# GiantAI/pixtrack

Hardware: AMD Instinct MI355X
Metric: tracked frames/sec at 640x480 (full NeRF render + UNet + LM loop) (higher is better)
Workload: dtype fp16 storage / fp32 accumulate (UNet, NeRF MLPs); fp32 (LM)

## Files before the change

include/pixtrack_hip.h:

```cpp
#ifndef PIXTRACK_HIP_H
#define PIXTRACK_HIP_H

#include <stdint.h>

#ifdef __cplusplus
extern "C" {
#endif

#define PXT_OK 0
#define PXT_E_ARG -1
#define PXT_E_HIP -2
#define PXT_E_TIMEOUT -3
#define PXT_E_STATE -4

#define PXT_MAX_LEVELS 8
#define PXT_LM_LOG_STRIDE 20

int pxt_version(void);
const char* pxt_last_error(void);
int pxt_device_cus(int* n_cus_host);

typedef struct {
  const float* fmap;
  const float* fref;
// ... 95 lines not shown
  float* out;
} pxt_lm_info_problem;
int64_t pxt_lm_information_workspace_bytes(int32_t n_problems);
int pxt_lm_information(const pxt_lm_info_problem* problems_host, int32_t n_problems, const pxt_lm_conf* conf_host,
                       void* workspace, void* stream);

#define PXT_LM_POINT_RECORD 8
#define PXT_LM_REPORT_SUMMARY 16
#define PXT_LM_REPORT_MAX_PROBLEMS 64
typedef struct {
  const float* p3d;
  const uint8_t* point_mask;
  int32_t n_points;
  pxt_lm_level level;
  const float* pose;
  int32_t pose_is_lm_record;
  float inlier_weight;
  float* points;
  float* summary;
} pxt_lm_report_problem;
int64_t pxt_lm_point_report_workspace_bytes(int32_t n_problems);
int pxt_lm_point_report(const pxt_lm_report_problem* problems_host, int32_t n_problems, const pxt_lm_conf* conf_host,
                        void* workspace, void* stream);

typedef struct pxt_unet pxt_unet;

int pxt_unet_create(const void* weights_host, int64_t n_bytes, pxt_unet** out_ctx);
int pxt_unet_destroy(pxt_unet* ctx);
int64_t pxt_unet_workspace_bytes(const pxt_unet* ctx, int32_t H, int32_t W);

int pxt_unet_activation_stats(pxt_unet* ctx, int32_t H, int32_t W, const void* workspace, float* stats_device ,
                              void* stream);

int pxt_unet_forward(pxt_unet* ctx, const void* image, int32_t image_is_u8, const uint8_t* mask,
                     int32_t H, int32_t W, float* const out_maps[3], const int32_t out_cstride[3],
                     int32_t normalize, void* workspace, void* stream);

#define PXT_UNET_MAX_BATCH 16
int64_t pxt_unet_workspace_bytes_batch(const pxt_unet* ctx, int32_t n_images, int32_t H, int32_t W);
int pxt_unet_forward_batch(pxt_unet* ctx, int32_t n_images, const void* const* images,
                           const int32_t* image_is_u8, const uint8_t* const* masks, int32_t H, int32_t W,
                           float* const* out_maps, const int32_t out_cstride[3], const int32_t* normalize,
                           void* workspace, void* stream);

int pxt_unet_set_tile_skip(pxt_unet* ctx, int32_t on);

int pxt_unet_set_batch_plan(pxt_unet* ctx, int32_t per_image_plan);

int64_t pxt_unet_workspace_bytes_pair(const pxt_unet* ctx, const int32_t H[2], const int32_t W[2]);
int pxt_unet_forward_pair(pxt_unet* ctx, const void* const* images, const int32_t* image_is_u8,
                          const uint8_t* const* masks, const int32_t H[2], const int32_t W[2],
                          float* const* out_maps, const int32_t out_cstride[3], const int32_t* normalize,
                          void* workspace, void* stream);
int pxt_unet_set_defer_join(pxt_unet* ctx, int32_t on);
int pxt_unet_pair_join(pxt_unet* ctx, void* stream);

int pxt_unet_create_f32(const void* weights_host, int64_t n_bytes, pxt_unet** out_ctx);
int pxt_unet_precision(const pxt_unet* ctx);


int pxt_conv3x3_nhwc_f16(const void* in, int32_t H, int32_t W, int32_t Cin, const void* weights,
                         const float* bias, int32_t Cout, int32_t relu, void* out, void* stream);

int pxt_conv3x3_nhwc_f32(const void* in, int32_t H, int32_t W, int32_t Cin, const void* weights,
                         const float* bias, int32_t Cout, int32_t relu, void* out, void* stream);

int64_t pxt_conv3x3_packed_bytes(int32_t Cin, int32_t Cout);
int pxt_conv3x3_pack_weights(const void* weights, int32_t Cin, int32_t Cout, void* packed, void* stream);
int pxt_conv3x3_packed(const void* in, int32_t H, int32_t W, int32_t Cin, const void* packed, const float* bias,
                       int32_t Cout, int32_t relu, void* out, void* pool_out, int32_t cfg, int32_t splits,
                       void* splitk_ws, int64_t splitk_ws_bytes, void* stream);

typedef struct pxt_ngp pxt_ngp;

typedef struct {
  int32_t n_levels, n_features, log2_hashmap, base_res;
  float per_level_scale;
  int32_t grid_cascades;
  float aabb_scale;
  float cone_angle;
  float depth_scale;
  int32_t linear_colors;
} pxt_ngp_model;

int pxt_ngp_create(const pxt_ngp_model* model_host, const void* grid_params_f16_host,
                   int64_t n_grid_params, const void* mlp_params_f16_host, int64_t n_mlp_params,
                   const uint8_t* occupancy_bits_host, int64_t n_occ_bytes, pxt_ngp** out_ctx);
int pxt_ngp_destroy(pxt_ngp* ctx);

typedef struct {
  float cam[12];
  float focal;
  float k1;
  float aabb_min[3], aabb_max[3];
  float background[4];
  float min_transmittance;
  int32_t width, height, spp;
  int32_t mode;
} pxt_ngp_view;

int pxt_ngp_render(pxt_ngp* ctx, const pxt_ngp_view* view_host, float* out_rgba,
                   uint64_t* stats ,
                   void* stream);

int pxt_ngp_render_both(pxt_ngp* ctx, const pxt_ngp_view* view_host, float* out_rgba, float* out_depth_rgba,
                        uint64_t* stats, void* stream);
// ... 77 lines not shown
```

pixtrack_amd/_lib.py:

```python
from __future__ import annotations

import ctypes as C
import os
from pathlib import Path
from typing import Optional

import torch

_HERE = Path(__file__).resolve().parent
LIB_PATH = Path(os.environ["PIXTRACK_HIP_LIB"]) if os.environ.get("PIXTRACK_HIP_LIB") else _HERE / "libpixtrack_hip.so"

PXT_MAX_LEVELS = 8
PXT_LM_LOG_STRIDE = 20
PXT_E_TIMEOUT = -3
ABI_VERSION = 13
PXT_LM_MAX_BATCH = 16
PXT_UNET_MAX_BATCH = 16
PXT_NGP_MAX_BATCH = 16
PXT_LM_INFO_RECORD = 48
PXT_LM_INFO_MAX_PROBLEMS = 64
PXT_LM_POINT_RECORD = 8
PXT_LM_REPORT_SUMMARY = 16
PXT_LM_REPORT_MAX_PROBLEMS = 64
PXT_POSE_ERR_RECORD = 8
# ... 8 lines not shown

class PxtError(RuntimeError):
    """Infrastructure failure of the native path (never a tracking failure)."""


class LmLevel(C.Structure):
    _fields_ = [
        ("fmap", C.c_void_p),
        ("fref", C.c_void_p),
        ("h", C.c_int32),
        ("w", C.c_int32),
        ("C", C.c_int32),
        ("cstride", C.c_int32),
        ("cam", C.c_float * 10),
        ("ndist", C.c_int32),
        ("lambda_", C.c_float * 6),
    ]


class LmConf(C.Structure):
    _fields_ = [
        ("num_iters", C.c_int32),
        ("pad", C.c_int32),
        ("loss", C.c_int32),
        ("loss_alpha", C.c_float),
        ("loss_scale", C.c_float),
        ("grad_stop", C.c_float),
        ("dt_stop", C.c_float),
        ("dR_stop", C.c_float),
        ("min_valid", C.c_int32),
        ("n_workgroups", C.c_int32),
        ("spin_limit", C.c_int32),
        ("path", C.c_int32),
    ]


class SampleLevel(C.Structure):
    _fields_ = [
        ("fmap", C.c_void_p),
        ("out", C.c_void_p),
        ("h", C.c_int32),
        ("w", C.c_int32),
        ("C", C.c_int32),
        ("cstride", C.c_int32),
        ("cam", C.c_float * 10),
        ("ndist", C.c_int32),
        ("x0", C.c_int32),
        ("y0", C.c_int32),
        ("full_w", C.c_int32),
        ("full_h", C.c_int32),
    ]


class NgpModel(C.Structure):
    _fields_ = [
        ("n_levels", C.c_int32),
        ("n_features", C.c_int32),
        ("log2_hashmap", C.c_int32),
        ("base_res", C.c_int32),
        ("per_level_scale", C.c_float),
        ("grid_cascades", C.c_int32),
        ("aabb_scale", C.c_float),
        ("cone_angle", C.c_float),
        ("depth_scale", C.c_float),
        ("linear_colors", C.c_int32),
    ]


class NgpView(C.Structure):
    _fields_ = [
        ("cam", C.c_float * 12),
        ("focal", C.c_float),
        ("k1", C.c_float),
        ("aabb_min", C.c_float * 3),
        ("aabb_max", C.c_float * 3),
        ("background", C.c_float * 4),
        ("min_transmittance", C.c_float),
        ("width", C.c_int32),
        ("height", C.c_int32),
        ("spp", C.c_int32),
        ("mode", C.c_int32),
    ]


class NgpOutputs(C.Structure):
    _fields_ = [("rgba", C.c_void_p), ("depth_rgba", C.c_void_p), ("rgb_u8", C.c_void_p), ("depth_nz", C.c_void_p)]


class LmCamera(C.Structure):
    _fields_ = [("conv27", C.c_double * 27), ("cam_slot", C.c_void_p * 2), ("cam_out13", C.c_void_p)]


class LmProblem(C.Structure):
    _fields_ = [("p3d", C.c_void_p), ("point_mask", C.c_void_p), ("n_points", C.c_int32),
                ("levels_host", C.POINTER(LmLevel)), ("n_levels", C.c_int32), ("T_init_host", C.POINTER(C.c_float)),
                ("out", C.c_void_p), ("log", C.c_void_p), ("workspace", C.c_void_p), ("cam_host", C.POINTER(LmCamera))]


class LmInfoProblem(C.Structure):
    _fields_ = [("p3d", C.c_void_p), ("point_mask", C.c_void_p), ("n_points", C.c_int32), ("level", LmLevel),
                ("pose", C.c_void_p), ("pose_is_lm_record", C.c_int32), ("out", C.c_void_p)]


class LmReportProblem(C.Structure):
    _fields_ = [("p3d", C.c_void_p), ("point_mask", C.c_void_p), ("n_points", C.c_int32), ("level", LmLevel),
                ("pose", C.c_void_p), ("pose_is_lm_record", C.c_int32), ("inlier_weight", C.c_float),
                ("points", C.c_void_p), ("summary", C.c_void_p)]


class RelocMap(C.Structure):
    _fields_ = [
        ("fmap", C.c_void_p),
        ("h", C.c_int32),
        ("w", C.c_int32),
        ("C", C.c_int32),
        ("cstride", C.c_int32),
        ("cam", C.c_float * 10),
        ("ndist", C.c_int32),
    ]


class RelocBank(C.Structure):
    _fields_ = [("p3d", C.c_void_p), ("fref", C.c_void_p), ("valid", C.c_void_p), ("n_points", C.c_int32)]


_lib: Optional[C.CDLL] = None

_VP, _I32, _I64 = C.c_void_p, C.c_int32, C.c_int64
PROTOTYPES = {
    "pxt_version": (C.c_int, []),
    "pxt_last_error": (C.c_char_p, []),
    "pxt_device_cus": (C.c_int, [C.POINTER(C.c_int)]),
    "pxt_lm_refine": (
        C.c_int,
        [_VP, _VP, _I32, C.POINTER(LmLevel), _I32, _VP, C.POINTER(LmConf), _VP, _VP, _VP, _VP],
    ),
    "pxt_lm_refine_cam": (
        C.c_int,
        [_VP, _VP, _I32, C.POINTER(LmLevel), _I32, _VP, C.POINTER(LmConf), _VP, _VP, _VP, C.POINTER(LmCamera), _VP],
    ),
    "pxt_lm_workspace_bytes": (_I64, []),
    "pxt_lm_batch_workspace_bytes": (_I64, [_I32]),
    "pxt_lm_refine_batch": (C.c_int, [C.POINTER(LmProblem), _I32, C.POINTER(LmConf), _VP, _VP]),
    "pxt_lm_information_workspace_bytes": (_I64, [_I32]),
    "pxt_lm_information": (C.c_int, [C.POINTER(LmInfoProblem), _I32, C.POINTER(LmConf), _VP, _VP]),
    "pxt_lm_point_report_workspace_bytes": (_I64, [_I32]),
    "pxt_lm_point_report": (C.c_int, [C.POINTER(LmReportProblem), _I32, C.POINTER(LmConf), _VP, _VP]),
    "pxt_sample_sparse": (C.c_int, [_VP, _I32, _VP, C.POINTER(SampleLevel), _I32, _I32, _I32, _VP, _VP]),
    "pxt_score_pose_hypotheses": (
        C.c_int, [C.POINTER(RelocMap), C.POINTER(RelocBank), _VP, _VP, _I32, C.POINTER(LmConf), _VP, _VP]),
    "pxt_unet_create": (C.c_int, [_VP, _I64, C.POINTER(_VP)]),
    "pxt_unet_create_f32": (C.c_int, [_VP, _I64, C.POINTER(_VP)]),
    "pxt_unet_precision": (C.c_int, [_VP]),
    "pxt_unet_destroy": (C.c_int, [_VP]),
    "pxt_unet_workspace_bytes": (_I64, [_VP, _I32, _I32]),
    "pxt_unet_forward": (
        C.c_int,
        [_VP, _VP, _I32, _VP, _I32, _I32, C.POINTER(_VP), C.POINTER(_I32), _I32, _VP, _VP],
    ),
    "pxt_unet_set_defer_join": (C.c_int, [_VP, _I32]),
    "pxt_unet_set_batch_plan": (C.c_int, [_VP, _I32]),
    "pxt_unet_set_tile_skip": (C.c_int, [_VP, _I32]),
    "pxt_unet_pair_join": (C.c_int, [_VP, _VP]),
    "pxt_unet_activation_stats": (C.c_int, [_VP, _I32, _I32, _VP, _VP, _VP]),
    "pxt_unet_workspace_bytes_batch": (_I64, [_VP, _I32, _I32, _I32]),
    "pxt_unet_forward_batch": (
        C.c_int,
        [_VP, _I32, C.POINTER(_VP), C.POINTER(_I32), C.POINTER(_VP), _I32, _I32, C.POINTER(_VP), C.POINTER(_I32),
         C.POINTER(_I32), _VP, _VP],
    ),
    "pxt_unet_workspace_bytes_pair": (_I64, [_VP, C.POINTER(_I32), C.POINTER(_I32)]),
    "pxt_unet_forward_pair": (
        C.c_int,
        [_VP, C.POINTER(_VP), C.POINTER(_I32), C.POINTER(_VP), C.POINTER(_I32), C.POINTER(_I32), C.POINTER(_VP),
         C.POINTER(_I32), C.POINTER(_I32), _VP, _VP],
    ),
    "pxt_conv3x3_nhwc_f16": (C.c_int, [_VP, _I32, _I32, _I32, _VP, _VP, _I32, _I32, _VP, _VP]),
    "pxt_conv3x3_nhwc_f32": (C.c_int, [_VP, _I32, _I32, _I32, _VP, _VP, _I32, _I32, _VP, _VP]),
    "pxt_conv3x3_packed_bytes": (_I64, [_I32, _I32]),
    "pxt_conv3x3_pack_weights": (C.c_int, [_VP, _I32, _I32, _VP, _VP]),
    "pxt_conv3x3_packed": (C.c_int, [_VP, _I32, _I32, _I32, _VP, _VP, _I32, _I32, _VP, _VP, _I32, _I32, _VP, _I64, _VP]),
    "pxt_ngp_create": (C.c_int, [C.POINTER(NgpModel), _VP, _I64, _VP, _I64, _VP, _I64, C.POINTER(_VP)]),
    "pxt_ngp_destroy": (C.c_int, [_VP]),
    "pxt_ngp_render": (C.c_int, [_VP, C.POINTER(NgpView), _VP, _VP, _VP]),
    "pxt_ngp_render_both": (C.c_int, [_VP, C.POINTER(NgpView), _VP, _VP, _VP, _VP]),
    "pxt_ngp_render_both_from_pose": (C.c_int, [_VP, C.POINTER(NgpView), _VP, C.POINTER(C.c_double), _VP, _VP, _VP, _VP, _VP]),
    "pxt_ngp_render_frame": (C.c_int, [_VP, C.POINTER(NgpView), _I32, _I32, C.POINTER(NgpOutputs), _VP, _VP]),
    "pxt_ngp_camera_slot": (_VP, [_VP]),
    "pxt_ngp_batch_workspace_bytes": (_I64, [_I32]),
    "pxt_ngp_render_frame_batch": (C.c_int, [C.POINTER(_VP), C.POINTER(NgpView), _I32, C.POINTER(_I32), _I32,
                                              C.POINTER(NgpOutputs), C.POINTER(_VP), _VP, _VP]),
    "pxt_ngp_create_shared": (C.c_int, [_VP, C.POINTER(_VP)]),
    "pxt_ngp_timing_enable": (C.c_int, [_VP, _I32]),
    "pxt_ngp_timing_read": (C.c_int, [_VP, C.POINTER(C.c_float), C.POINTER(_I32)]),
    "pxt_ngp_query": (C.c_int, [_VP, _VP, _VP, _I32, _VP, _VP]),
    "pxt_depth_mask": (C.c_int, [_VP, _I32, _I32, _I32, _I32, _VP, _VP, _VP]),
    "pxt_depth_mask_plane": (C.c_int, [_VP, _I32, _I32, _I32, _I32, _VP, _VP, _VP]),
    "pxt_rgba_to_u8": (C.c_int, [_VP, _I32, _I32, C.c_float, _VP, _VP]),
    "pxt_resize_linear": (C.c_int, [_VP, _I32, _I32, _I32, _VP, _I32, _I32, _VP]),
    "pxt_resize_activity": (C.c_int, [_VP, _VP, _I32, _I32, _I32, _I32, _VP, _VP]),
    "pxt_points_from_depth_workspace_bytes": (_I64, [_I32, _I32]),
    "pxt_points_from_depth": (C.c_int, [_VP, _I32, _I32, C.POINTER(C.c_float), C.c_float, C.c_float, C.c_float, _I32, _I32,
                                        _VP, _VP, _VP, _VP, _VP]),
    "pxt_pose_errors_workspace_bytes": (_I64, [_I32, _I32]),
    "pxt_pose_errors": (C.c_int, [_VP, _I32, _VP, _I32, _I32, _VP, _VP, _VP]),
    "pxt_depth_agreement_workspace_bytes": (_I64, [_I32, _I32, _I32]),
    "pxt_depth_agreement": (C.c_int, [_VP, _VP, _I32, _I32, _I32, C.c_float, C.POINTER(C.c_float), _I32, _VP, _VP, _VP]),
    "pxt_symmetric_pose_errors_workspace_bytes": (_I64, [_I32, _I32, _I32]),
    "pxt_symmetric_pose_errors": (C.c_int, [_VP, _I32, _VP, _I32, _VP, _I32, _VP, _VP, _VP]),
    "pxt_sensor_vsd_workspace_bytes": (_I64, [_I32, _I32, _I32]),
    "pxt_sensor_vsd": (C.c_int, [_VP, _VP, _VP, _VP, _I32, _I32, _I32, _I32, _I32, C.c_float, C.c_float, C.c_float,
                                 C.POINTER(C.c_float), _I32, _VP, _VP, _VP]),
# ... 56 lines not shown
```

pixtrack_amd/csrc/pxt_common.h:

```cpp
#pragma once

#include <hip/hip_runtime.h>
#include <stdint.h>

#include "../../include/pixtrack_hip.h"

#define PXT_WAVE 64

namespace pxt {

void set_last_error(const char* what, hipError_t e);
hipStream_t shared_side_stream(int i);
#define PXT_HIP_CHECK(expr)                         \
  do {                                              \
    hipError_t _e = (expr);                         \
    if (_e != hipSuccess) {                         \
      ::pxt::set_last_error(#expr, _e);             \
      return PXT_E_HIP;                             \
    }                                               \
  } while (0)

struct Cam {
  float w, h, fx, fy, cx, cy, k1, k2, p1, p2;
  int ndist;
};

__host__ __device__ inline Cam make_cam(const float* c10, int ndist) {
  Cam c;
  c.w = c10[0]; c.h = c10[1]; c.fx = c10[2]; c.fy = c10[3]; c.cx = c10[4]; c.cy = c10[5];
  c.k1 = c10[6]; c.k2 = c10[7]; c.p1 = c10[8]; c.p2 = c10[9];
  c.ndist = ndist;
  return c;
}

constexpr float kCamEps = 1e-3f;

__device__ inline bool project_point(const Cam& c, float x, float y, float z, float& u, float& v,
                                     float* J ) {
  bool visible = z > kCamEps;
  float zc = fmaxf(z, kCamEps);
  float iz = 1.0f / zc;
  float xn = x * iz, yn = y * iz;
  float xd = xn, yd = yn;
  bool dist_ok = true;
  float Jd00 = 1.f, Jd01 = 0.f, Jd10 = 0.f, Jd11 = 1.f;
  if (c.ndist > 0) {
    float r2 = xn * xn + yn * yn;
    float radial = c.k1 * r2 + c.k2 * r2 * r2;
    xd = xn + xn * radial;
    yd = yn + yn * radial;
    float disc = 9.f * c.k1 * c.k1 - 20.f * c.k2;
    bool limited = ((c.k2 > 0.f) && (disc > 0.f)) || ((c.k2 <= 0.f) && (c.k1 > 0.f));
    if (limited) {
      float limit = (c.k2 > 0.f) ? (sqrtf(fmaxf(disc, 0.f)) - 3.f * c.k1) / (10.f * c.k2)
                                 : 1.f / (3.f * c.k1);
      dist_ok = r2 < fabsf(limit);
    }
    float uv = xn * yn;
    float d_radial = 2.f * c.k1 + 4.f * c.k2 * r2;
    Jd00 += radial + xn * xn * d_radial;
    Jd11 += radial + yn * yn * d_radial;
    Jd01 += uv * d_radial;
    Jd10 += uv * d_radial;
    if (c.ndist > 2) {
      xd += 2.f * c.p1 * uv + c.p2 * (r2 + 2.f * xn * xn);
      yd += 2.f * c.p2 * uv + c.p1 * (r2 + 2.f * yn * yn);
      Jd00 += 2.f * c.p1 * yn + 6.f * c.p2 * xn;
      Jd11 += 2.f * c.p2 * xn + 6.f * c.p1 * yn;
      Jd01 += 2.f * c.p1 * xn + 2.f * c.p2 * yn;
      Jd10 += 2.f * c.p2 * yn + 2.f * c.p1 * xn;
    }
  }
  u = xd * c.fx + c.cx;
  v = yd * c.fy + c.cy;
  bool in_img = (u >= 0.f) && (v >= 0.f) && (u <= c.w - 1.f) && (v <= c.h - 1.f);
  if (J) {
    float a = iz, bx = -x * iz * iz, by = -y * iz * iz;
    float m00 = c.fx * Jd00, m01 = c.fx * Jd01, m10 = c.fy * Jd10, m11 = c.fy * Jd11;
    J[0] = m00 * a; J[1] = m01 * a; J[2] = m00 * bx + m01 * by;
    J[3] = m10 * a; J[4] = m11 * a; J[5] = m10 * bx + m11 * by;
  }
  return visible && dist_ok && in_img;
}

template <int WIDTH>
__device__ inline float group_allreduce_sum(float v) {
#pragma unroll
  for (int m = 1; m < WIDTH; m <<= 1) v += __shfl_xor(v, m, PXT_WAVE);
  return v;
}
// ... 113 lines not shown
```

pixtrack_amd/csrc/pxt_conv_v2.h:

```cpp
#pragma once

#include <type_traits>

namespace pxt {

constexpr int kV2RowBytes = 1280;
constexpr int kV2Cols = 18;

struct FusedHead {
  const half8* wfrag;
  const float* conf_w;
  const float* bias;
  float* out[PXT_UNET_MAX_BATCH];
  int normalize[PXT_UNET_MAX_BATCH];
  int cstride, enabled;
};

struct FusedFirst {
  const void* image[PXT_UNET_MAX_BATCH];
  const uint8_t* mask[PXT_UNET_MAX_BATCH];
  int is_u8[PXT_UNET_MAX_BATCH];
  const float* w;
  const float* b;
  int enabled;
};

struct TileSkip {
  const uint8_t* flags;
  const half_t* value;
};

template <int TH, int BNC, int NT>
__device__ __forceinline__ void conv_fill_constant_tile(const half_t* __restrict__ value, half_t* __restrict__ out_img,
                                                        half_t* __restrict__ pool_img, int H, int W, int Cout, int ty0, int tx0,
                                                        int co0) {
  constexpr int CH = BNC / 8;
  const half8* cv = (const half8*)(value + co0);
  for (int i = threadIdx.x; i < TH * 16 * CH; i += NT) {
    const int c = i % CH, p = i / CH;
    const int y = ty0 + (p >> 4), x = tx0 + (p & 15);
    if (y < H && x < W) *(half8*)(out_img + ((size_t)y * W + x) * Cout + co0 + 8 * c) = cv[c];
  }
  if (pool_img) {
    const int Hp = H >> 1, Wp = W >> 1;
    for (int i = threadIdx.x; i < (TH / 2) * 8 * CH; i += NT) {
      const int c = i % CH, p = i / CH;
      const int y = (ty0 >> 1) + (p >> 3), x = (tx0 >> 1) + (p & 7);
      if (y < Hp && x < Wp) *(half8*)(pool_img + ((size_t)y * Wp + x) * Cout + co0 + 8 * c) = cv[c];
    }
  }
}

struct ConvArgs {
  const half_t* in;
  int H, W, Cin;
  const half_t* wpk;
  const float* bias;
  int Cout, relu;
  half_t* out;
  float* partial;
  UpSrc up;
  half_t* pool;
  FusedHead head;
  FusedFirst first;
  TileSkip skip;
};

__host__ __device__ inline size_t packed_weight_index(int cout, int tap, int cin, int Cout) {
  const int k = cin & 31, s = k >> 4, lane = (cout & 31) + 32 * ((k & 15) >> 3), j = k & 7;
  return ((((size_t)(cin >> 5) * 9 + tap) * 2 + s) * (size_t)(Cout >> 5) + (cout >> 5)) * 512 + lane * 8 + j;
}

__global__ void pack_conv_weights_kernel(const half_t* __restrict__ w , int Cin, int Cout,
                                         half_t* __restrict__ packed) {
  const long long i = (long long)blockIdx.x * blockDim.x + threadIdx.x;
  if (i >= (long long)Cout * 9 * Cin) return;
  const int cin = (int)(i % Cin);
  const int tap = (int)((i / Cin) % 9);
  const int cout = (int)(i / ((long long)Cin * 9));
  packed[packed_weight_index(cout, tap, cin, Cout)] = w[i];
}

typedef __attribute__((ext_vector_type(2))) _Float16 half2v;

template <int I, int N, class F>
__device__ __forceinline__ void static_for(F&& f) {
  if constexpr (I < N) {
    f(std::integral_constant<int, I>{});
    static_for<I + 1, N>(f);
  }
}

__device__ inline int opaque(int x) {
  asm volatile("" : "+v"(x));
  return x;
}

__device__ inline unsigned pool2x2_pk(unsigned v) {
  auto sw = __builtin_amdgcn_permlane16_swap(v, v, false, false);
  half2v a = __builtin_bit_cast(half2v, (unsigned)sw[0]), b = __builtin_bit_cast(half2v, (unsigned)sw[1]);
  half2v m = __builtin_elementwise_max(a, b);
  const unsigned mu = __builtin_bit_cast(unsigned, m);
  const unsigned nb = (unsigned)__builtin_amdgcn_update_dpp((int)mu, (int)mu, 0xB1 , 0xF, 0xF, false);
  m = __builtin_elementwise_max(m, __builtin_bit_cast(half2v, nb));
  return __builtin_bit_cast(unsigned, m);
}

#if PXT_EXP_STAMPS
__device__ unsigned long long pxt_stamps[8192 * 16];
#define PXT_STAMP(k)                                                                              \
  do {                                                                                            \
    if (threadIdx.x == 0) {                                                                       \
      const unsigned wg_ = blockIdx.x + gridDim.x * (blockIdx.y + gridDim.y * blockIdx.z);        \
      if (wg_ < 8192) pxt_stamps[wg_ * 16 + (k)] = __builtin_amdgcn_s_memtime();                 \
      if (wg_ < 8192 && ((k) == 0 || (k) == 3))                                                   \
        pxt_stamps[wg_ * 16 + ((k) == 0 ? 14 : 15)] = __builtin_amdgcn_s_memrealtime();          \
    }                                                                                             \
  } while (0)
#else
#define PXT_STAMP(k)
#endif
template <int CW, int PBW, int WC, int WP, bool UPCAT, int AR = 3, bool FIRST = false>
__global__ __launch_bounds__(256, AR > 3 ? 1 : 2) void conv3x3_v2_kernel(const ConvArgs a) {
  static_assert(!FIRST || !UPCAT, "the fused first layer feeds a plain layer");
  static_assert(18 % AR == 0, "the ring is indexed by the step modulo AR at compile time");
  static_assert(WC * WP == 4, "four waves per workgroup");
  constexpr int TH = 2 * PBW * WP, HR = TH + 2;
  constexpr int BNC = 32 * CW * WC;
  constexpr int kElems = HR * kV2Cols * 4;
  constexpr int KH = (kElems + 255) / 256;
  constexpr int NB = 2;
  constexpr int KB = (KH + NB - 1) / NB;
  constexpr int kBuf = HR * kV2RowBytes;
  extern __shared__ __attribute__((aligned(16))) char smem[];

  PXT_STAMP(0);
  const int tid = threadIdx.x;
  const int lane = tid & 63;
  const int wave = __builtin_amdgcn_readfirstlane(tid >> 6);
  const int wc = wave / WP, wp = wave % WP;
  const int H = a.H, W = a.W, Cin = a.Cin, Cout = a.Cout;
  const int tiles_x = (W + 15) >> 4;
  const int tiles_per = tiles_x * ((H + TH - 1) / TH);
  const int img = blockIdx.x / tiles_per, tile = blockIdx.x % tiles_per;
  const int n_img = gridDim.x / tiles_per;
  const int ty0 = (tile / tiles_x) * TH, tx0 = (tile % tiles_x) * 16;
  const int co0 = blockIdx.y * BNC;
  const int Cs = UPCAT ? Cin - a.up.Cp : Cin;
  const int in_w = UPCAT ? a.up.Ws : W;
  const half_t* in = a.in + (size_t)img * (UPCAT ? a.up.Hs : H) * in_w * Cs;
  const half_t* prev = UPCAT ? a.up.prev + (size_t)img * a.up.Hp * a.up.Wp * a.up.Cp : nullptr;
  if (a.skip.flags != nullptr && a.skip.flags[blockIdx.x] == 0) {
    conv_fill_constant_tile<TH, BNC, 256>(a.skip.value, a.out + (size_t)img * H * W * Cout,
                                          a.pool ? a.pool + (size_t)img * (H >> 1) * (W >> 1) * Cout : nullptr, H, W, Cout, ty0,
                                          tx0, co0);
    return;
  }

  float* const s_bias = (float*)(smem + 2 * kBuf + (UPCAT ? (PBW * WP + 2) * 10 * 64 : 0));
  if (tid < BNC) s_bias[tid] = a.bias[co0 + tid];

  f32x16 acc[CW][PBW];
#pragma unroll
  for (int c = 0; c < CW; ++c)
#pragma unroll
    for (int p = 0; p < PBW; ++p)
#pragma unroll
      for (int r = 0; r < 16; ++r) acc[c][p][r] = 0.f;

  const int r31 = lane & 31, khalf = lane >> 5;
  int boff[3][2];
#pragma unroll
  for (int kx = 0; kx < 3; ++kx)
#pragma unroll
    for (int s = 0; s < 2; ++s) {
      const int col = (r31 & 15) + kx;
      boff[kx][s] = (2 * PBW * wp + (r31 >> 4)) * kV2RowBytes + col * 64 + (((2 * s + khalf) ^ ((col >> 2) & 3)) << 4);
    }

  const int n_chunks = Cin >> 5;
  const int per_z = (n_chunks + (int)gridDim.z - 1) / (int)gridDim.z;
  const int ch_begin = (int)blockIdx.z * per_z, ch_end = min(n_chunks, ch_begin + per_z);

  const size_t a_step = (size_t)(Cout >> 5) * 512;
  const half_t* aptr = a.wpk + ((size_t)ch_begin * 18) * a_step + (size_t)((co0 >> 5) + CW * wc) * 512 + lane * 8;

  half8 r_in[KB];
  unsigned goff[KH];
#pragma unroll
  for (int k = 0; k < KH; ++k) {
    const int i = tid + 256 * k;
    const int pix = i >> 2, seg = i & 3;
    const int gy = ty0 + pix / kV2Cols - 1, gx = tx0 + pix % kV2Cols - 1;
    const bool ok = i < kElems && gy >= 0 && gy < H && gx >= 0 && gx < W;
    goff[k] = ok ? ((unsigned)(gy * in_w + gx) * (unsigned)Cs + (unsigned)(seg * 8)) * 2u : 0x80000000u;
  }
  const __amdgpu_buffer_rsrc_t in_rsrc = __builtin_amdgcn_make_buffer_rsrc(
      (void*)in, 0, (int)((size_t)(UPCAT ? a.up.Hs : H) * in_w * Cs * 2), 0x00020000);
  const int cp0 = UPCAT ? a.up.Cp : 0;
  auto halo_issue = [&](int c0, int batch) {
#pragma unroll
    for (int kk = 0; kk < KB; ++kk) {
      const int k = batch * KB + kk;
      if (k < KH)
        r_in[kk] = __builtin_bit_cast(half8, __builtin_amdgcn_raw_buffer_load_b128(
                                                 in_rsrc, (int)(goff[k] + (unsigned)((c0 - cp0) * 2)), 0, 0));
    }
  };
  auto halo_write = [&](int buf, int batch) {
    const int t_ = opaque(tid);
#pragma unroll
    for (int kk = 0; kk < KB; ++kk) {
      const int k = batch * KB + kk;
      const int i = t_ + 256 * k;
      const int pix = i >> 2, seg = i & 3;
      const int hy = pix / kV2Cols, hx = pix % kV2Cols;
      if (k < KH && i < kElems)
        *(half8*)(smem + buf * kBuf + hy * kV2RowBytes + hx * 64 + ((seg ^ ((hx >> 2) & 3)) << 4)) = r_in[kk];
    }
  };

  constexpr int PH = TH / 2 + 2, PW = 10;
  constexpr int kPatchElems = PH * PW * 4, KP = (kPatchElems + 255) / 256;
  static_assert(!UPCAT || KP <= KB, "the patch pieces reuse the halo staging registers");
  char* const patch = smem + 2 * kBuf;
  unsigned poff[UPCAT ? KP : 1], up_src[UPCAT ? KH : 1];
  if (UPCAT) {
    const int py0 = (ty0 >> 1) - 1, px0 = (tx0 >> 1) - 1;
#pragma unroll
    for (int kp = 0; kp < KP; ++kp) {
      const int i = min(tid + 256 * kp, kPatchElems - 1);
      const int pp = i >> 2, seg = i & 3;
      const int sy = min(max(py0 + pp / PW, 0), a.up.Hp - 1), sx = min(max(px0 + pp % PW, 0), a.up.Wp - 1);
      poff[kp] = (unsigned)(sy * a.up.Wp + sx) * (unsigned)a.up.Cp + (unsigned)(seg * 8);
    }
#pragma unroll
    for (int k = 0; k < KH; ++k) {
      const int i = tid + 256 * k;
      const int pix = i >> 2, seg = i & 3;
      const int gy = ty0 + pix / kV2Cols - 1, gx = tx0 + pix % kV2Cols - 1;
      const bool ok = i < kElems && gy >= 0 && gy < H && gx >= 0 && gx < W;
      const float sy = fmaxf(((float)gy + 0.5f) * 0.5f - 0.5f, 0.f);
      const float sx = fmaxf(((float)gx + 0.5f) * 0.5f - 0.5f, 0.f);
      const int y0 = min((int)sy, a.up.Hp - 1), x0 = min((int)sx, a.up.Wp - 1);
      const int y1 = min(y0 + 1, a.up.Hp - 1), x1 = min(x0 + 1, a.up.Wp - 1);
      const float ay = sy - (float)y0, ax = sx - (float)x0;
      const int pidx = ok ? (y0 - py0) * PW + (x0 - px0) : 0;
      up_src[k] = ((unsigned)(pidx * 64 + seg * 16) << 8) | (ok ? 64u : 0u) | (x1 != x0 ? 1u : 0u) | (y1 != y0 ? 2u : 0u) |
                  (ax == 0.25f ? 4u : ax == 0.75f ? 8u : 0u) | (ay == 0.25f ? 16u : ay == 0.75f ? 32u : 0u);
    }
  }
  auto patch_issue = [&](int c0) {
#pragma unroll
    for (int kp = 0; kp < KP; ++kp) r_in[kp] = *(const half8*)(prev + (poff[UPCAT ? kp : 0] + (unsigned)c0));
  };
  auto patch_write = [&]() {
    const int t_ = opaque(tid);
#pragma unroll
    for (int kp = 0; kp < KP; ++kp) {
      const int i = t_ + 256 * kp;
      if (i < kPatchElems) *(half8*)(patch + i * 16) = r_in[kp];
    }
  };
  auto patch_interp = [&](int buf) {
    const int t_ = opaque(tid);
#pragma unroll
    for (int k = 0; k < KH; ++k) {
      const int i = t_ + 256 * k;
      const int pix = i >> 2, seg = i & 3;
      const int hy = pix / kV2Cols, hx = pix % kV2Cols;
      const unsigned f = (unsigned)opaque((int)up_src[UPCAT ? k : 0]);
      const char* src = patch + (f >> 8);
      const int dx = (f & 1u) ? 64 : 0, dy = (f & 2u) ? PW * 64 : 0;
      const float ax = (f & 4u) ? 0.25f : (f & 8u) ? 0.75f : 0.f;
      const float ay = (f & 16u) ? 0.25f : (f & 32u) ? 0.75f : 0.f;
      const half8 p00 = *(const half8*)(src), p01 = *(const half8*)(src + dx);
      const half8 p10 = *(const half8*)(src + dy), p11 = *(const half8*)(src + dy + dx);
      const bool ok_ = (f & 64u) != 0;
      const half_t wa = (half_t)(ok_ ? (1.f - ax) * (1.f - ay) : 0.f), wb = (half_t)(ok_ ? ax * (1.f - ay) : 0.f);
      const half_t wc = (half_t)(ok_ ? (1.f - ax) * ay : 0.f), wd = (half_t)(ok_ ? ax * ay : 0.f);
      half8 v = p00 * wa;
// ... 287 lines not shown
```

pixtrack_amd/csrc/pxt_conv_v3.h:

```cpp
#pragma once

namespace pxt {

template <int KC>
struct V3Geo {
  static constexpr int kPix = KC * 2;
  static constexpr int kNP = KC / 8;
  static constexpr int kRow = 20 * kPix;
  static constexpr int kPixPerBankRow = 256 / kPix;
  __device__ static inline int swz(int col) {
    return kPixPerBankRow == 4 ? ((col >> 2) & 3) : ((col >> 3) & 1);
  }
};

__host__ __device__ inline size_t packed_weight_index_v3(int cout, int tap, int cin, int Cout) {
  const int ky = tap / 3, kx = tap % 3;
  const int k = cin & 31, s = k >> 4, lane = (cout & 31) + 32 * ((k & 15) >> 3), j = k & 7;
  const size_t group = (size_t)(cin >> 5) * 6 + s * 3 + kx;
  return ((group * 3 + ky) * (size_t)(Cout >> 5) + (cout >> 5)) * 512 + lane * 8 + j;
}

__global__ void pack_conv_weights_v3_kernel(const half_t* __restrict__ w , int Cin, int Cout,
                                            half_t* __restrict__ packed) {
  const long long i = (long long)blockIdx.x * blockDim.x + threadIdx.x;
// ... 4 lines not shown
  packed[packed_weight_index_v3(cout, tap, cin, Cout)] = w[i];
}

__device__ inline unsigned pk_max(unsigned a, unsigned b) {
  return __builtin_bit_cast(unsigned, __builtin_elementwise_max(__builtin_bit_cast(half2v, a), __builtin_bit_cast(half2v, b)));
}

constexpr int v3_lds_bytes(int CW, int PBW, int WC, int WP, int KC, bool upcat = false, int KS = 1) {
  return KS * (2 * (2 * PBW * WP + 2) * (20 * KC * 2) + 2 * 3 * CW * WC * 1024) + 32 * CW * WC * 4 +
         (upcat ? (PBW * WP + 2) * 10 * KC * 2 : 0);
}

template <int CW, int PBW, int WC, int WP, int KC, bool UPCAT = false, int KS = 1>
__global__ __launch_bounds__(256 * KS, 2) void conv3x3_v3_kernel(const ConvArgs a) {
  static_assert(WC * WP == 4, "four waves per quartet");
  static_assert(KS == 1 || (KS == 2 && !UPCAT), "K split across two wave quartets: plain layers only");
  static_assert(KC == 16 || KC == 32, "chunk of 16 or 32 input channels");
  using G = V3Geo<KC>;
  constexpr int TH = 2 * PBW * WP, HR = TH + 2;
  constexpr int NCB = CW * WC, BNC = 32 * NCB;
  constexpr int NG = 3 * (KC / 16);
  constexpr int kBuf = HR * G::kRow;
  constexpr int kABuf = 3 * NCB * 1024;
  constexpr int kElems = HR * kV2Cols * G::kNP;
  constexpr int KH = (kElems + 255) / 256;
  constexpr int kAElems = 3 * NCB * 64;
  constexpr int KA = (kAElems + 255) / 256;
  extern __shared__ __attribute__((aligned(16))) char smem[];
  constexpr int kQuartet = 2 * kBuf + 2 * kABuf;
  const int kh = KS == 1 ? 0 : __builtin_amdgcn_readfirstlane((int)threadIdx.x >> 8);
  char* const s_halo = smem + kh * kQuartet;
  char* const s_a = s_halo + 2 * kBuf;
  float* const s_bias = (float*)(smem + KS * kQuartet);
  char* const patch = smem + KS * kQuartet + BNC * 4;

  PXT_STAMP(0);
  const int tid = threadIdx.x & 255;
  const int lane = tid & 63;
  const int wave = __builtin_amdgcn_readfirstlane(tid >> 6);
  const int wc = wave / WP, wp = wave % WP;
  const int H = a.H, W = a.W, Cin = a.Cin, Cout = a.Cout;
  const int tiles_x = (W + 15) >> 4;
  const int tiles_per = tiles_x * ((H + TH - 1) / TH);
  const int img = blockIdx.x / tiles_per, tile = blockIdx.x % tiles_per;
  const int n_img = gridDim.x / tiles_per;
  const int ty0 = (tile / tiles_x) * TH, tx0 = (tile % tiles_x) * 16;
  const int co0 = blockIdx.y * BNC;
  const int Cs = UPCAT ? Cin - a.up.Cp : Cin;
  const int in_w = UPCAT ? a.up.Ws : W;
  const int cp0 = UPCAT ? a.up.Cp : 0;
  const half_t* in = a.in + (size_t)img * (UPCAT ? a.up.Hs : H) * in_w * Cs;
  const half_t* prev = UPCAT ? a.up.prev + (size_t)img * a.up.Hp * a.up.Wp * a.up.Cp : nullptr;
  if (a.skip.flags != nullptr && a.skip.flags[blockIdx.x] == 0) {
    conv_fill_constant_tile<TH, BNC, 256 * KS>(a.skip.value, a.out + (size_t)img * H * W * Cout,
                                               a.pool ? a.pool + (size_t)img * (H >> 1) * (W >> 1) * Cout : nullptr, H, W, Cout,
                                               ty0, tx0, co0);
    return;
  }

  if ((int)threadIdx.x < BNC) s_bias[threadIdx.x] = a.bias[co0 + threadIdx.x];

  f32x16 acc[CW][PBW];
#pragma unroll
  for (int c = 0; c < CW; ++c)
#pragma unroll
    for (int p = 0; p < PBW; ++p)
#pragma unroll
      for (int r = 0; r < 16; ++r) acc[c][p][r] = 0.f;

  const int r31 = lane & 31, khalf = lane >> 5;
  const int lrow = 2 * PBW * wp + (r31 >> 4) * PBW, lcol = r31 & 15;

  const int n_chunks = Cin / KC;
  const int per_z = (n_chunks + (int)gridDim.z - 1) / (int)gridDim.z;
  int ch_begin = (int)blockIdx.z * per_z, ch_end = min(n_chunks, ch_begin + per_z);
  if (KS == 2) {
    const int half = (ch_end - ch_begin) >> 1;
    ch_begin += kh * half;
    ch_end = ch_begin + half;
  }
  const int n_groups = (ch_end - ch_begin) * NG;

  const size_t a_group = (size_t)3 * (Cout >> 5) * 512;
  const half_t* const wbase = a.wpk + (size_t)ch_begin * NG * a_group + (size_t)(co0 >> 5) * 512;
  unsigned a_src[KA];
#pragma unroll
  for (int k = 0; k < KA; ++k) {
    const int i = min(tid + 256 * k, kAElems - 1);
    const int ky = i / (NCB * 64), rem = i % (NCB * 64);
    a_src[k] = (unsigned)(ky * (Cout >> 5) * 512 + rem * 8);
  }
  half8 r_a[KA];
  const half_t* a_next = wbase;
  auto a_issue_piece = [&](auto k_c) {
    constexpr int k = decltype(k_c)::value;
    r_a[k] = *(const half8*)(a_next + a_src[k]);
  };
  auto a_write_piece = [&](auto k_c, int buf) {
    constexpr int k = decltype(k_c)::value;
    const int i = opaque(tid) + 256 * k;
    if (i < kAElems) *(half8*)(s_a + buf * kABuf + i * 16) = r_a[k];
  };

  half8 r_in[KH];
  unsigned goff[KH];
#pragma unroll
  for (int k = 0; k < KH; ++k) {
    const int i = tid + 256 * k;
    const int pix = i / G::kNP, seg = i % G::kNP;
    const int gy = ty0 + pix / kV2Cols - 1, gx = tx0 + pix % kV2Cols - 1;
    const bool ok = i < kElems && gy >= 0 && gy < H && gx >= 0 && gx < W;
    goff[k] = ok ? ((unsigned)(gy * in_w + gx) * (unsigned)Cs + (unsigned)(seg * 8)) * 2u : 0x80000000u;
  }
  const __amdgpu_buffer_rsrc_t in_rsrc = __builtin_amdgcn_make_buffer_rsrc(
      (void*)in, 0, (int)((size_t)(UPCAT ? a.up.Hs : H) * in_w * Cs * 2), 0x00020000);
  auto halo_issue_piece = [&](auto k_c, int c0) {
    constexpr int k = decltype(k_c)::value;
    r_in[k] = __builtin_bit_cast(half8, __builtin_amdgcn_raw_buffer_load_b128(in_rsrc, (int)(goff[k] + (unsigned)((c0 - cp0) * 2)), 0, 0));
  };
  auto halo_write_piece = [&](auto k_c, int buf) {
    constexpr int k = decltype(k_c)::value;
    const int i = opaque(tid) + 256 * k;
    const int pix = i / G::kNP, seg = i % G::kNP;
    const int hy = pix / kV2Cols, hx = pix % kV2Cols;
    if (i < kElems) *(half8*)(s_halo + buf * kBuf + hy * G::kRow + hx * G::kPix + ((seg ^ G::swz(hx)) << 4)) = r_in[k];
  };

  constexpr int PH = TH / 2 + 2, PW = 10;
  constexpr int kPatchElems = PH * PW * G::kNP, KP = (kPatchElems + 255) / 256;
  static_assert(!UPCAT || KP <= KH, "the patch pieces reuse the halo staging registers");
  unsigned poff[UPCAT ? KP : 1], up_src[UPCAT ? KH : 1];
  if constexpr (UPCAT) {
    const int py0 = (ty0 >> 1) - 1, px0 = (tx0 >> 1) - 1;
#pragma unroll
    for (int kp = 0; kp < KP; ++kp) {
      const int i = min(tid + 256 * kp, kPatchElems - 1);
      const int pp = i / G::kNP, seg = i % G::kNP;
      const int sy = min(max(py0 + pp / PW, 0), a.up.Hp - 1), sx = min(max(px0 + pp % PW, 0), a.up.Wp - 1);
      poff[kp] = (unsigned)(sy * a.up.Wp + sx) * (unsigned)a.up.Cp + (unsigned)(seg * 8);
    }
#pragma unroll
    for (int k = 0; k < KH; ++k) {
      const int i = tid + 256 * k;
      const int pix = i / G::kNP, seg = i % G::kNP;
      const int gy = ty0 + pix / kV2Cols - 1, gx = tx0 + pix % kV2Cols - 1;
      const bool ok = i < kElems && gy >= 0 && gy < H && gx >= 0 && gx < W;
      const float sy = fmaxf(((float)gy + 0.5f) * 0.5f - 0.5f, 0.f);
      const float sx = fmaxf(((float)gx + 0.5f) * 0.5f - 0.5f, 0.f);
      const int y0 = min((int)sy, a.up.Hp - 1), x0 = min((int)sx, a.up.Wp - 1);
      const int y1 = min(y0 + 1, a.up.Hp - 1), x1 = min(x0 + 1, a.up.Wp - 1);
      const float ay = sy - (float)y0, ax = sx - (float)x0;
      const int pidx = ok ? (y0 - py0) * PW + (x0 - px0) : 0;
      up_src[k] = ((unsigned)(pidx * G::kPix + seg * 16) << 8) | (ok ? 64u : 0u) | (x1 != x0 ? 1u : 0u) | (y1 != y0 ? 2u : 0u) |
                  (ax == 0.25f ? 4u : ax == 0.75f ? 8u : 0u) | (ay == 0.25f ? 16u : ay == 0.75f ? 32u : 0u);
    }
  }
  auto patch_issue_piece = [&](auto k_c, int c0) {
    constexpr int k = decltype(k_c)::value;
    if constexpr (UPCAT && k < KP) r_in[k] = *(const half8*)(prev + (poff[k] + (unsigned)c0));
  };
  auto patch_write_piece = [&](auto k_c) {
    constexpr int k = decltype(k_c)::value;
    if constexpr (UPCAT && k < KP) {
      const int i = opaque(tid) + 256 * k;
      if (i < kPatchElems) *(half8*)(patch + i * 16) = r_in[k];
    }
  };
  auto patch_interp_piece = [&](auto k_c, int buf) {
    constexpr int k = decltype(k_c)::value;
    if constexpr (UPCAT) {
      const int i = opaque(tid) + 256 * k;
      const int pix = i / G::kNP, seg = i % G::kNP;
      const int hy = pix / kV2Cols, hx = pix % kV2Cols;
      const unsigned f = (unsigned)opaque((int)up_src[k]);
      const char* src = patch + (f >> 8);
      const int dx = (f & 1u) ? G::kPix : 0, dy = (f & 2u) ? PW * G::kPix : 0;
      const float ax = (f & 4u) ? 0.25f : (f & 8u) ? 0.75f : 0.f;
      const float ay = (f & 16u) ? 0.25f : (f & 32u) ? 0.75f : 0.f;
      const half8 p00 = *(const half8*)(src), p01 = *(const half8*)(src + dx);
      const half8 p10 = *(const half8*)(src + dy), p11 = *(const half8*)(src + dy + dx);
      const bool ok_ = (f & 64u) != 0;
      const half_t wa = (half_t)(ok_ ? (1.f - ax) * (1.f - ay) : 0.f), wb = (half_t)(ok_ ? ax * (1.f - ay) : 0.f);
      const half_t wc = (half_t)(ok_ ? (1.f - ax) * ay : 0.f), wd = (half_t)(ok_ ? ax * ay : 0.f);
      half8 v = p00 * wa;
      v = p01 * wb + v;
      v = p10 * wc + v;
// ... 282 lines not shown
```

pixtrack_amd/csrc/pxt_lm.hip:

```cpp
#include "pxt_common.h"
#include "pxt_lm_point.h"

#include <algorithm>

namespace pxt {

constexpr int kLmBlock = 512;
constexpr int kLmWaves = kLmBlock / PXT_WAVE;
constexpr int kLmMaxGrid = 256;
constexpr int kNAcc = 32;
constexpr int kGrpStride = 33;
constexpr unsigned kSpinLimit = 1u << 22;

struct LmLevelDev {
  const float* fmap;
  const float* fref;
  int h, w, C, cs;
  float cam[10];
  int ndist;
  float lambda[6];
};

struct LmGrid {
  int G, b;
// ... 656 lines not shown
        __hip_atomic_store(&P.cam_out[12], 1.f, __ATOMIC_RELEASE, __HIP_MEMORY_SCOPE_SYSTEM);
      }
    }
  }
}

__global__ __launch_bounds__(kLmBlock) void lm_refine_kernel(const LmParams P) {
  __shared__ LmShared sh;
  lm_refine_problem(P, LmGrid{(int)gridDim.x, (int)blockIdx.x}, sh);
}

__global__ __launch_bounds__(kLmBlock) void lm_refine_batch_kernel(const LmParams* __restrict__ params, const int K,
                                                                   const int contiguous) {
  __shared__ LmShared sh;
  const int G = (int)gridDim.x / K;
  const int p = contiguous ? (int)blockIdx.x / G : (int)blockIdx.x % K;
  const int b = contiguous ? (int)blockIdx.x % G : (int)blockIdx.x / K;
  lm_refine_problem(params[p], LmGrid{G, b}, sh);
}

struct SampleLevelDev {
  const float* fmap;
  float* out;
  int h, w, C, cs;
  float cam[10];
  int ndist;
  int x0, y0, fw, fh;
};

struct SampleParams {
  const float* p3d;
  float T[12];
  int n, n_levels, pad, normalize;
  SampleLevelDev lv[PXT_MAX_LEVELS];
  uint8_t* valid;
};

template <int LG>
__device__ inline bool sample_level(const SampleParams& P, const SampleLevelDev& L, int n,
                                    bool active, float px, float py, float pz, int sub) {
  const Cam cam = make_cam(L.cam, L.ndist);
  const int W = L.w, H = L.h, C = L.C, cs = L.cs;
  const int FW = L.fw, FH = L.fh;
  const float pad = (float)P.pad;
  float u = 0.f, v = 0.f;
  bool valid = active;
  point_in_window(cam, px, py, pz, valid, FW, FH, pad, u, v, nullptr);
  if (!active) return false;
  float* o = L.out + (size_t)n * cs;
  if (!valid) {
    for (int c0 = 4 * sub; c0 < cs; c0 += 4 * LG) *(float4*)(o + c0) = make_float4(0, 0, 0, 0);
    return false;
  }
  const float fu = floorf(u), fv = floorf(v);
  const int ix0f = (int)fu, iy0f = (int)fv;
  const float ax = u - fu, ay = v - fv;
  const int x1f = min(ix0f + 1, FW - 1), y1f = min(iy0f + 1, FH - 1);
  const float mx = (ix0f + 1 < FW) ? 1.f : 0.f, my = (iy0f + 1 < FH) ? 1.f : 0.f;
  const float w00 = (1.f - ax) * (1.f - ay), w10 = ax * (1.f - ay) * mx, w01 = (1.f - ax) * ay * my,
              w11 = ax * ay * mx * my;
  const int ix0 = min(max(ix0f - L.x0, 0), W - 1), iy0 = min(max(iy0f - L.y0, 0), H - 1);
  const int x1 = min(max(x1f - L.x0, 0), W - 1), y1 = min(max(y1f - L.y0, 0), H - 1);
  const float* p00 = L.fmap + ((size_t)iy0 * W + ix0) * cs;
  const float* p10 = L.fmap + ((size_t)iy0 * W + x1) * cs;
  const float* p01 = L.fmap + ((size_t)y1 * W + ix0) * cs;
  const float* p11 = L.fmap + ((size_t)y1 * W + x1) * cs;
  float ss = 0.f;
  for (int c0 = 4 * sub; c0 < C; c0 += 4 * LG) {
    float4 a = *(const float4*)(p00 + c0), b = *(const float4*)(p10 + c0),
           c = *(const float4*)(p01 + c0), d = *(const float4*)(p11 + c0);
    float4 f;
    f.x = w00 * a.x + w10 * b.x + w01 * c.x + w11 * d.x;
    f.y = w00 * a.y + w10 * b.y + w01 * c.y + w11 * d.y;
    f.z = w00 * a.z + w10 * b.z + w01 * c.z + w11 * d.z;
    f.w = w00 * a.w + w10 * b.w + w01 * c.w + w11 * d.w;
    ss += f.x * f.x + f.y * f.y + f.z * f.z + f.w * f.w;
    *(float4*)(o + c0) = f;
  }
  ss = group_allreduce_sum<LG>(ss);
  if (P.normalize) {
    const float inv = 1.f / fmaxf(sqrtf(ss), 1e-12f);
    for (int c0 = 4 * sub; c0 < C; c0 += 4 * LG) {
      float4 f = *(float4*)(o + c0);
      f.x *= inv; f.y *= inv; f.z *= inv; f.w *= inv;
      *(float4*)(o + c0) = f;
    }
  }
  if (sub == 0) {
    o[C] = w00 * p00[C] + w10 * p10[C] + w01 * p01[C] + w11 * p11[C];
    for (int c = C + 1; c < cs; ++c) o[c] = 0.f;
  }
  return true;
}

__global__ __launch_bounds__(256) void sample_sparse_kernel(const SampleParams P) {
  constexpr int LG = 32;
  constexpr int GPW = PXT_WAVE / LG;
  const int lane = threadIdx.x & (PXT_WAVE - 1);
  const int sub = lane % LG, grp = lane / LG;
  const int wave_global = (blockIdx.x * blockDim.x + threadIdx.x) / PXT_WAVE;
  const int n = wave_global * GPW + grp;
  const bool active = n < P.n;
  float X = 0.f, Y = 0.f, Z = 1.f;
  if (active) {
    X = P.p3d[3 * n];
    Y = P.p3d[3 * n + 1];
    Z = P.p3d[3 * n + 2];
  }
  float px, py, pz;
  transform_point(P.T, X, Y, Z, px, py, pz);
  bool all_valid = active;
  for (int l = 0; l < P.n_levels; ++l)
    all_valid = sample_level<LG>(P, P.lv[l], n, active, px, py, pz, sub) && all_valid;
  if (active && sub == 0) P.valid[n] = all_valid ? 1 : 0;
}
// ... 185 lines not shown
```

pixtrack_amd/csrc/pxt_lm_point.h:

```cpp
#pragma once

#include "pxt_common.h"

namespace pxt {

__device__ inline void robust_loss(int kind, float alpha, float scale, float x, float& loss,
                                   float& w) {
  if (kind == 0) {
    loss = x;
    w = 1.f;
    return;
  }
  float a2 = scale * scale;
  float y = x / a2;
  float l, d;
  if (kind == 1) {
    if (y <= 1.f) {
      l = y;
      d = 1.f;
    } else {
      float sy = sqrtf(y);
      l = 2.f * sy - 1.f;
      d = fmaxf(1.1920929e-07f, 1.f / sy);
    }
// ... 3 lines not shown
      d = 2.f / (y + 2.f);
    } else if (alpha == 2.f) {
      l = y;
      d = 1.f;
    } else {
      float beta = fmaxf(fabsf(alpha - 2.f), 1e-7f);
      float as = (alpha >= 0.f ? 1.f : -1.f) * fmaxf(fabsf(alpha), 1e-7f);
      l = 2.f * (beta / as) * (powf(y / beta + 1.f, 0.5f * alpha) - 1.f);
      d = powf(y / beta + 1.f, 0.5f * alpha - 1.f);
    }
  }
  loss = l * a2;
  w = d;
}

__device__ inline float lm_dpp_add(float v, int ctrl_tag) {
  const int iv = __builtin_bit_cast(int, v);
  int o;
  if (ctrl_tag == 0) o = __builtin_amdgcn_update_dpp(iv, iv, 0xB1, 0xF, 0xF, false);
  else if (ctrl_tag == 1) o = __builtin_amdgcn_update_dpp(iv, iv, 0x4E, 0xF, 0xF, false);
  else if (ctrl_tag == 2) o = __builtin_amdgcn_update_dpp(iv, iv, 0x141, 0xF, 0xF, false);
  else o = __builtin_amdgcn_update_dpp(iv, iv, 0x140, 0xF, 0xF, false);
  return v + __builtin_bit_cast(float, o);
}

__device__ inline float lm_group_sum(float v, bool wide) {
  v = lm_dpp_add(v, 0);
  v = lm_dpp_add(v, 1);
  v = lm_dpp_add(v, 2);
  if (wide) {
    v = lm_dpp_add(v, 3);
    v += __shfl_xor(v, 16, PXT_WAVE);
  }
  return v;
}

template <int LG>
__device__ inline float lm_group_sum_t(float v) {
  v = lm_dpp_add(v, 0);
  v = lm_dpp_add(v, 1);
  v = lm_dpp_add(v, 2);
  if (LG >= 16) v = lm_dpp_add(v, 3);
  if (LG >= 32) v += __shfl_xor(v, 16, PXT_WAVE);
  return v;
}

__device__ inline float lm_row16_sum(float v) {
  v = lm_dpp_add(v, 0);
  v = lm_dpp_add(v, 1);
  v = lm_dpp_add(v, 2);
  return lm_dpp_add(v, 3);
}

__device__ inline void transform_point(const float* T, float X, float Y, float Z, float& px, float& py, float& pz) {
  px = T[0] * X + T[1] * Y + T[2] * Z + T[9];
  py = T[3] * X + T[4] * Y + T[5] * Z + T[10];
  pz = T[6] * X + T[7] * Y + T[8] * Z + T[11];
}

__device__ inline void point_in_window(const Cam& cam, float px, float py, float pz, bool& valid, int W, int H, float pad,
                                       float& u, float& v, float* Jw ) {
  valid = project_point(cam, px, py, pz, u, v, Jw) && valid;
  valid = valid && (u >= pad) && (v >= pad) && (u <= (float)(W - 1) - pad) && (v <= (float)(H - 1) - pad);
}

__device__ inline void bilinear_weights(float u, float v, int& ix0, int& iy0, float& w00, float& w10, float& w01,
                                        float& w11) {
  const float fu = floorf(u), fv = floorf(v);
  ix0 = (int)fu;
  iy0 = (int)fv;
  const float ax = u - fu, ay = v - fv;
  w00 = (1.f - ax) * (1.f - ay);
  w10 = ax * (1.f - ay);
  w01 = (1.f - ax) * ay;
  w11 = ax * ay;
}

#define PXT_LM_POINT_CH(w00_, w10_, w01_, w11_, a01_, a02_, a10_, a11_, a12_, a13_, a20_, a21_, a22_, a23_, a31_, a32_, \
                        f_, s_cost_, A0_, A1_, B00_, B01_, B11_)                                                        \
  {                                                                                                                     \
    const float a01 = (a01_), a02 = (a02_), a10 = (a10_), a11 = (a11_), a12 = (a12_), a13 = (a13_), a20 = (a20_),       \
                a21 = (a21_), a22 = (a22_), a23 = (a23_), a31 = (a31_), a32 = (a32_);                                   \
    const float F = (w00_) * a11 + (w10_) * a12 + (w01_) * a21 + (w11_) * a22;                                          \
    const float Fxp = (w00_) * a12 + (w10_) * a13 + (w01_) * a22 + (w11_) * a23;                                        \
    const float Fxm = (w00_) * a10 + (w10_) * a11 + (w01_) * a20 + (w11_) * a21;                                        \
    const float Fyp = (w00_) * a21 + (w10_) * a22 + (w01_) * a31 + (w11_) * a32;                                        \
    const float Fym = (w00_) * a01 + (w10_) * a02 + (w01_) * a11 + (w11_) * a12;                                        \
    const float gx = 0.5f * (Fxp - Fxm), gy = 0.5f * (Fyp - Fym);                                                       \
    const float r = F - (f_);                                                                                           \
    (s_cost_) += r * r;                                                                                                 \
    (A0_) += r * gx;                                                                                                    \
    (A1_) += r * gy;                                                                                                    \
    (B00_) += gx * gx;                                                                                                  \
    (B01_) += gx * gy;                                                                                                  \
    (B11_) += gy * gy;                                                                                                  \
  }

#define PXT_LM_POINT_CH_COST(w00_, w10_, w01_, w11_, a11_, a12_, a21_, a22_, f_, s_cost_)    \
  {                                                                                          \
    const float a11 = (a11_), a12 = (a12_), a21 = (a21_), a22 = (a22_);                      \
    const float F = (w00_) * a11 + (w10_) * a12 + (w01_) * a21 + (w11_) * a22;               \
    const float r = F - (f_);                                                                \
    (s_cost_) += r * r;                                                                      \
  }

__device__ inline void point_jacobian(const float* Jw, float px, float py, float pz, float* J0, float* J1) {
  J0[0] = Jw[0]; J0[1] = Jw[1]; J0[2] = Jw[2];
  J1[0] = Jw[3]; J1[1] = Jw[4]; J1[2] = Jw[5];
  J0[3] = -Jw[1] * pz + Jw[2] * py;
  J0[4] = Jw[0] * pz - Jw[2] * px;
  J0[5] = -Jw[0] * py + Jw[1] * px;
  J1[3] = -Jw[4] * pz + Jw[5] * py;
  J1[4] = Jw[3] * pz - Jw[5] * px;
  J1[5] = -Jw[3] * py + Jw[4] * px;
}

template <bool ADD>
__device__ __forceinline__ void point_normal_terms(float* dst, float wgt, const float* J0, const float* J1, float A0,
                                                   float A1, float B00, float B01, float B11) {
  float M0[6], M1[6];
#pragma unroll
  for (int k = 0; k < 6; ++k) {
    M0[k] = B00 * J0[k] + B01 * J1[k];
    M1[k] = B01 * J0[k] + B11 * J1[k];
    dst[k] = (ADD ? dst[k] : 0.f) + wgt * (J0[k] * A0 + J1[k] * A1);
  }
  int idx = 6;
#pragma unroll
// ... 7 lines not shown
```

pixtrack_amd/csrc/pxt_unet.hip:

```cpp
#include "pxt_common.h"
#include "pxt_unet_f32.h"

#include <algorithm>
#include <array>
#include <cstdio>
#include <cstdlib>
#include <cstring>
#include <utility>
#include <vector>

namespace pxt {

typedef _Float16 half_t;
typedef __attribute__((ext_vector_type(8))) _Float16 half8;
typedef __attribute__((ext_vector_type(4))) _Float16 half4;
typedef __attribute__((ext_vector_type(16))) float f32x16;

constexpr int kNumConv = 17;
constexpr int kNumHeads = 3;

constexpr int kFW = 64, kFH = 4;
struct FirstImages {
  const void* image[PXT_UNET_MAX_BATCH];
  const uint8_t* mask[PXT_UNET_MAX_BATCH];
  int is_u8[PXT_UNET_MAX_BATCH];
};

template <int COUT>
__global__ __launch_bounds__(256) void conv_first_kernel(const FirstImages imgs, int H, int W,
                                                         const float* __restrict__ wts,
                                                         const float* __restrict__ bias,
                                                         half_t* __restrict__ out) {
  __shared__ float s_px[(kFH + 2) * (kFW + 2) * 3];
  __shared__ __attribute__((aligned(16))) half_t s_out[kFH * kFW * COUT];
  const int im = blockIdx.y;
  const void* image = imgs.image[im];
  const uint8_t* mask = imgs.mask[im];
  const bool u8 = imgs.is_u8[im] != 0;
  out += (size_t)im * H * W * COUT;
  const int tiles_x = (W + kFW - 1) / kFW;
  const int tx0 = (blockIdx.x % tiles_x) * kFW, ty0 = (blockIdx.x / tiles_x) * kFH;
  const float mean[3] = {0.485f, 0.456f, 0.406f};
  const float istd[3] = {1.f / 0.229f, 1.f / 0.224f, 1.f / 0.225f};
  for (int i = threadIdx.x; i < (kFH + 2) * (kFW + 2); i += 256) {
    const int hy = i / (kFW + 2), hx = i % (kFW + 2);
    const int yy = ty0 + hy - 1, xx = tx0 + hx - 1;
    const bool ok = yy >= 0 && yy < H && xx >= 0 && xx < W;
    float m = 1.f;
    if (ok && mask) m = (float)mask[(size_t)yy * W + xx];
#pragma unroll
    for (int c = 0; c < 3; ++c) {
      float v = 0.f;
      if (ok) {
// ... 282 lines not shown
      else for (int x = 0; x < n; ++x) any |= p[x];
    } else {
      const uint8_t* p = u8 + ((size_t)y * W + x0) * 3;
      if (n == 8 && (((uintptr_t)p) & 7) == 0) {
        const unsigned long long* q = (const unsigned long long*)p;
        any = (q[0] | q[1] | q[2]) != 0ull;
      } else {
        for (int x = 0; x < 3 * n; ++x) any |= p[x];
      }
    }
  }
  any |= __shfl_xor(any, 1, 64);
  any |= __shfl_xor(any, 2, 64);
  any |= __shfl_xor(any, 4, 64);
  if (live && r == 0) grid[(size_t)img * bh * bw + b] = any ? 1 : 0;
}

struct SkipLayerGeo {
  int th, shift, radius, h, w, offset;
};
struct SkipGeo {
  SkipLayerGeo l[6];
  int n_layers;
};
__global__ void skip_tile_flags_kernel(const SkipGeo geo, const uint8_t* __restrict__ grid, int H, int W, int bh, int bw,
                                       int n_img, uint8_t* __restrict__ flags) {
  const SkipLayerGeo g = geo.l[blockIdx.y];
  const int tiles_x = (g.w + 15) >> 4, tiles_y = (g.h + g.th - 1) / g.th;
  const int t = (blockIdx.x * blockDim.x + threadIdx.x) >> 6, lane = threadIdx.x & 63;
  if (t >= n_img * tiles_x * tiles_y) return;
  const int img = t / (tiles_x * tiles_y), tile = t % (tiles_x * tiles_y);
  const int ty0 = (tile / tiles_x) * g.th, tx0 = (tile % tiles_x) * 16;
  const int y0 = (ty0 << g.shift) - g.radius, y1 = (min(ty0 + g.th, g.h) << g.shift) + g.radius;
  const int x0 = (tx0 << g.shift) - g.radius, x1 = (min(tx0 + 16, g.w) << g.shift) + g.radius;
  unsigned any = (y0 < 0 || x0 < 0 || y1 > H || x1 > W) ? 1u : 0u;
  if (!any) {
    const uint8_t* gi = grid + (size_t)img * bh * bw;
    const int by0 = y0 >> 3, bx0 = x0 >> 3, nby = ((y1 - 1) >> 3) - by0 + 1, nbx = ((x1 - 1) >> 3) - bx0 + 1;
    for (int c = lane; c < nby * nbx; c += 64) any |= gi[(by0 + c / nbx) * bw + bx0 + c % nbx];
  }
  any = __ballot(any != 0) != 0ull;
  if (lane == 0) flags[g.offset + t] = any ? 1 : 0;
}

__global__ void skip_fill_kernel(half_t* __restrict__ dst, int n_pix, int C, const half_t* __restrict__ value) {
  const int i = blockIdx.x * blockDim.x + threadIdx.x;
  if (i < n_pix * C) dst[i] = value[i % C];
}
__global__ void skip_copy_kernel(half_t* __restrict__ dst, const half_t* __restrict__ src, int C) {
  const int i = blockIdx.x * blockDim.x + threadIdx.x;
  if (i < C) dst[i] = src[i];
}

struct UnetLayer {
  int cin, cout;
  const void* w;
  const float* b;
};

}

struct pxt_unet {
  pxt::UnetF32* f32 = nullptr;
  void* dev_head = nullptr;
  const pxt::half_t* head_w[pxt::kNumHeads];
  const float* head_b[pxt::kNumHeads];
  void* dev_blob = nullptr;
  void* dev_head0 = nullptr;
  void* dev_packed = nullptr;
  const pxt::half_t* conv_packed[pxt::kNumConv];
  int64_t n_bytes = 0;
  struct SideSet {
    hipStream_t side = nullptr;
    hipEvent_t ev_enc4 = nullptr, ev_dec1 = nullptr, ev_side = nullptr;
  } sides[2];
  hipStream_t pass2 = nullptr;
  hipEvent_t ev_fork = nullptr, ev_join = nullptr;
  struct SkipEntry {
    int cfg[6] = {0, 0, 0, 0, 0, 0};
    unsigned long long stamp = 0;
    pxt::half_t* values = nullptr;
  } skip_cache[8];
  unsigned long long skip_clock = 0;
  bool tile_skip = true;
  void* skip_scratch = nullptr;
  bool plan_as_single = false;
  bool defer_join = false;
  bool join_pending = false;
  pxt::UnetLayer conv[pxt::kNumConv];
  pxt::UnetLayer head[pxt::kNumHeads];
};

using namespace pxt;

namespace {

inline int env_int(const char* name, int dflt) { const char* e = getenv(name); return e ? atoi(e) : dflt; }
std::vector<std::array<int, 3>> parse_plan(const char* e) {
  std::vector<std::array<int, 3>> v;
  for (; e && *e; e = strchr(e, ';') ? strchr(e, ';') + 1 : nullptr) {
    std::array<int, 3> t = {0, 0, 0};
    if (sscanf(e, "%d:%d:%d", &t[0], &t[1], &t[2]) >= 2) v.push_back(t);
  }
  return v;
}
struct Knobs {
  int streams = env_int("PXT_UNET_STREAMS", 2);
  bool merge_heads = env_int("PXT_UNET_MERGE_HEADS", 1) != 0;
  bool skip = env_int("PXT_UNET_SKIP", 1) != 0;
  bool fuse_first = env_int("PXT_UNET_FUSE_FIRST", 1) != 0;
  const char* plan_env = getenv("PXT_CONV_PLAN");
  std::vector<std::array<int, 3>> plan = parse_plan(plan_env);
  bool debug = getenv("PXT_CONV_DEBUG") != nullptr;
};
const Knobs& knobs() { static const Knobs k; return k; }

struct EncBlock { int first, n, cin, c; };
constexpr int kNumEncLayers = 13;
constexpr EncBlock kEnc[5] = {{0, 2, 3, 64}, {2, 2, 64, 128}, {4, 3, 128, 256}, {7, 3, 256, 512}, {10, 3, 512, 512}};
inline int enc_block(int li) { int b = 4; while (kEnc[b].first > li) --b; return b; }
inline bool enc_last(int li) { return li == kEnc[enc_block(li)].first + kEnc[enc_block(li)].n - 1; }

inline bool fuses_first(const pxt_unet* ctx) { return knobs().fuse_first && ctx->conv[1].cin == 64 && ctx->conv[1].cout == 64; }

struct TileCfg {
  int kernel;
  int CW, PBW, WC, WP, KC, KS;
  int upcat_c;
  bool pool;
  int twin;
  bool deep;
  bool first;
};
constexpr int kNumCfgs = 22;
constexpr TileCfg kTileCfgs[kNumCfgs] = {
    {},
    {2, 2, 4, 2, 2, 32, 1, 0, true, 0, true, false},
    {2, 2, 2, 1, 4, 32, 1, 64, true, 0, false, true},
    {},
    {2, 2, 2, 2, 2, 32, 1, 0, true, 0, false, false},
    {},
    {2, 1, 2, 1, 4, 32, 1, 32, true, 0, false, false},
    {}, {}, {}, {},
    {3, 2, 4, 2, 2, 32, 1, 0, true, 0, false, false},
    {},
    {3, 2, 4, 1, 4, 16, 1, 0, true, 0, false, false},
    {3, 2, 2, 2, 2, 32, 1, 0, true, 0, false, false},
    {3, 2, 3, 2, 2, 32, 1, 0, false, 0, false, false},
    {3, 1, 4, 1, 4, 16, 1, 32, true, 0, false, false},
    {3, 2, 3, 1, 4, 16, 1, 64, false, 0, false, false},
    {3, 2, 3, 2, 2, 32, 2, 0, false, 15, false, false},
    {3, 2, 4, 2, 2, 32, 2, 0, true, 11, false, false},
    {3, 1, 2, 1, 4, 16, 1, 32, true, 0, false, false},
    {3, 2, 2, 1, 4, 16, 1, 64, true, 0, false, false}};
inline bool cfg_valid(int cfg) { return cfg >= 1 && cfg < kNumCfgs && kTileCfgs[cfg].kernel != 0; }
inline int cfg_th(int cfg) { return 2 * kTileCfgs[cfg].PBW * kTileCfgs[cfg].WP; }
inline int cfg_bnc(int cfg) { return 32 * kTileCfgs[cfg].CW * kTileCfgs[cfg].WC; }
inline const half_t* cfg_taps(int cfg, const half_t* wpk, int cin, int cout) {
  return kTileCfgs[cfg].kernel == 3 ? wpk + (size_t)cout * 9 * cin : wpk;
}

struct ConvPlan { int cfg, tiles, nb, splits; };

// ... 14 lines not shown
                   int force_splits, bool upcat, bool wants_pool) {
  ConvPlan P;
  const int plan_img = sc.single ? 1 : n_img, plan_peers = sc.single ? 2 : sc.peers;
  auto wgs_of = [&](int cfg) {
    const int th = cfg_th(cfg);
    return plan_peers * plan_img * ((H + th - 1) / th) * ((W + 15) / 16) * (cout / cfg_bnc(cfg));
  };
  int cfg = force_cfg;
  if (!cfg_valid(cfg) || cout % cfg_bnc(cfg) != 0) {
    if (cout % 128 == 0) {
      cfg = wgs_of(4) >= 512 ? 4 : 1;
      const int w15 = wgs_of(15);
      if (!wants_pool && w15 >= 192 && w15 <= 512) cfg = 15;
      const bool even_k = (cin / 32) % 2 == 0;
      if (cfg == 15 && w15 <= 256 && even_k) cfg = 18;
      if (cfg == 1 && wgs_of(1) <= 256 && wgs_of(1) >= 128 && even_k) cfg = 19;
      if (cfg == 1 && allow_split && wgs_of(15) < 192 && (cin / 32) % 8 == 0) cfg = 18;
    }
    else if (cout % 64 == 0) cfg = 2;
    else cfg = 6;
  }
  if (cfg_valid(cfg) && kTileCfgs[cfg].KS == 2 && (upcat || (cin / 32) % 2 != 0)) cfg = kTileCfgs[cfg].twin;
  P.cfg = cfg;
  const int th = cfg_th(cfg);
  P.tiles = n_img * ((H + th - 1) / th) * ((W + 15) / 16);
  P.nb = cout / cfg_bnc(cfg);
  const int plan_tiles = P.tiles / n_img * plan_img;
  P.splits = allow_split ? (force_splits > 0 ? std::min(force_splits, std::max(1, cin / 32)) : choose_splits(plan_peers * plan_tiles * P.nb, cin / 32, upcat, plan_tiles * P.nb)) : 1;
  if (kTileCfgs[cfg].KS == 2) {
    while (P.splits > 1 && (cin / 32) % (2 * P.splits) != 0) --P.splits;
  }
  return P;
}

inline int upcat_cfg(int cout, int H, int W) {
  return cout % 64 == 0 ? ((long long)H * W >= 120 * 160 ? 21 : 2) : 20;
}

size_t splitk_bytes(int n_img, int H, int W, int cin, int cout, bool upcat = false) {
  int splits = 1;
  for (int single = 0; single < 2; ++single)
    for (int peers = 1; peers <= 2; ++peers)
      for (int pool = 0; pool < (upcat ? 1 : 2); ++pool)
        splits = std::max(splits, plan_conv(PlanScope{peers, single != 0, 0}, n_img, H, W, cin, cout, true,
                                            upcat ? upcat_cfg(cout, H, W) : 0, 0, upcat, pool != 0).splits);
  return splits > 1 ? (size_t)splits * n_img * H * W * cout * sizeof(float) : 0;
}

struct Plan {
  int h[5], w[5];
  int dh[4], dw[4];
  size_t enc_tmp[5][2], enc_pool[5], enc_out[5], dec_out[4], splitk, splitk_bytes, total;
  size_t skip_grid, skip_flags;
  int skip_bh, skip_bw;
};

inline size_t align256(size_t x) { return (x + 255) / 256 * 256; }

bool make_plan(const pxt_unet* ctx, int n_img, int H, int W, Plan& P) {
  if (n_img < 1 || n_img > PXT_UNET_MAX_BATCH) return false;
  P.h[0] = H; P.w[0] = W;
  for (int b = 1; b < 5; ++b) { P.h[b] = P.h[b - 1] / 2; P.w[b] = P.w[b - 1] / 2; }
  if (P.h[4] < 1 || P.w[4] < 1) return false;
  int ph = P.h[4], pw = P.w[4];
  for (int d = 0; d < 4; ++d) { ph *= 2; pw *= 2; P.dh[d] = ph; P.dw[d] = pw; }
  size_t off = 0;
  auto take = [&](size_t bytes) { size_t o = off; off = align256(off + bytes); return o; };
  for (int b = 0; b < 5; ++b) {
    const size_t px = (size_t)n_img * P.h[b] * P.w[b];
    P.enc_pool[b] = (b > 0) ? take(px * kEnc[b].cin * 2) : 0;
    P.enc_tmp[b][0] = take(px * kEnc[b].c * 2);
    P.enc_tmp[b][1] = take(px * kEnc[b].c * 2);
    P.enc_out[b] = take(px * kEnc[b].c * 2);
  }
  for (int d = 0; d < 4; ++d) {
    const size_t px = (size_t)n_img * P.dh[d] * P.dw[d];
    P.dec_out[d] = take(px * ctx->conv[13 + d].cout * 2);
  }
  size_t sk = 0;
  for (int i = 1; i < kNumEncLayers; ++i)
    sk = std::max(sk, splitk_bytes(n_img, P.h[enc_block(i)], P.w[enc_block(i)], ctx->conv[i].cin, ctx->conv[i].cout));
  for (int d = 0; d < 4; ++d)
    sk = std::max(sk, splitk_bytes(n_img, P.dh[d], P.dw[d], ctx->conv[13 + d].cin, ctx->conv[13 + d].cout, true));
  P.splitk = take(sk + 256);
  P.splitk_bytes = sk;
  P.skip_bh = (H + 7) / 8;
  P.skip_bw = (W + 7) / 8;
  P.skip_grid = take((size_t)n_img * P.skip_bh * P.skip_bw);
  P.skip_flags = take((size_t)n_img * 6 * ((size_t)(H / 8 + 2) * (W / 16 + 2)));
  P.total = off;
  return true;
}

inline size_t enc_out_offset(const Plan& P, int li) {
  return enc_last(li) ? P.enc_out[enc_block(li)] : P.enc_tmp[enc_block(li)][(li - kEnc[enc_block(li)].first) & 1];
}

template <auto K, int LDS>
void launch_with_lds(const ConvArgs& a, dim3 grid, int threads, hipStream_t s) {
  static const hipError_t attr = hipFuncSetAttribute((const void*)K, hipFuncAttributeMaxDynamicSharedMemorySize, LDS);
  (void)attr;
  hipLaunchKernelGGL(K, grid, dim3(threads), LDS, s, a);
}

template <int CW, int PBW, int WC, int WP, bool UPCAT, int AR = 3, bool FIRST = false>
void launch_v2(const ConvArgs& a, dim3 grid, hipStream_t s) {
  constexpr int lds = 2 * (2 * PBW * WP + 2) * kV2RowBytes + (UPCAT ? (PBW * WP + 2) * 10 * 64 : 0) + 32 * CW * WC * 4 +
                      (FIRST ? (2 * PBW * WP + 4) * 20 * 3 * 4 : 0);
  launch_with_lds<conv3x3_v2_kernel<CW, PBW, WC, WP, UPCAT, AR, FIRST>, lds>(a, grid, 256, s);
}

template <int CW, int PBW, int WC, int WP, int KC, bool UPCAT = false, int KS = 1>
void launch_v3(const ConvArgs& a, dim3 grid, hipStream_t s) {
  constexpr int lds = v3_lds_bytes(CW, PBW, WC, WP, KC, UPCAT, KS);
  launch_with_lds<conv3x3_v3_kernel<CW, PBW, WC, WP, KC, UPCAT, KS>, lds>(a, grid, 256 * KS, s);
}

template <size_t C>
void launch_tile(bool upcat, bool deep, const ConvArgs& a, dim3 grid, hipStream_t s) {
  constexpr TileCfg T = kTileCfgs[C];
  if constexpr (T.kernel == 3) {
    if constexpr (T.upcat_c != 0) { if (upcat) return launch_v3<T.CW, T.PBW, T.WC, T.WP, T.KC, true>(a, grid, s); }
    launch_v3<T.CW, T.PBW, T.WC, T.WP, T.KC, false, T.KS>(a, grid, s);
  } else if constexpr (T.kernel == 2) {
    if constexpr (T.upcat_c != 0) { if (upcat) return launch_v2<T.CW, T.PBW, T.WC, T.WP, true>(a, grid, s); }
    if constexpr (T.deep) { if (deep) return launch_v2<T.CW, T.PBW, T.WC, T.WP, false, 9>(a, grid, s); }
    if constexpr (T.first) { if (a.first.enabled) return launch_v2<T.CW, T.PBW, T.WC, T.WP, false, 3, true>(a, grid, s); }
    launch_v2<T.CW, T.PBW, T.WC, T.WP, false>(a, grid, s);
  }
}

template <size_t... C>
constexpr auto tile_launches(std::index_sequence<C...>) { return std::array{&launch_tile<C>...}; }
constexpr auto kTileLaunches = tile_launches(std::make_index_sequence<kNumCfgs>());

int launch_tile_cfg(int cfg, bool upcat, const PlanScope& sc, const ConvArgs& a, dim3 grid, hipStream_t s) {
  if (!cfg_valid(cfg) || (upcat && kTileCfgs[cfg].upcat_c == 0)) return PXT_E_ARG;
  const bool deep = (long long)sc.peers * grid.x * grid.y * grid.z <= 256;
  kTileLaunches[cfg](upcat, deep, a, grid, s);
  return PXT_OK;
}

struct ConvLaunch {
  const half_t* in = nullptr;
  half_t* out = nullptr;
  int H = 0, W = 0, cin = 0, cout = 0, n_img = 1, relu = 1;
  const half_t* wpk = nullptr;
  const float* bias = nullptr;
  float* partial = nullptr;
  size_t partial_cap = ~(size_t)0;
  const UpSrc* up = nullptr;
  half_t* pool_out = nullptr;
  int force_cfg = 0, force_splits = 0, skip_cfg = 0;
  const FusedHead* head = nullptr;
  const FusedFirst* first = nullptr;
  const TileSkip* skip = nullptr;
};

ConvPlan resolve_plan(const ConvLaunch& L, const PlanScope& sc) {
  int force_cfg = L.force_cfg, force_splits = L.force_splits;
  for (const auto& t : knobs().plan)
    if (t[0] == sc.layer && sc.layer > 0) {
      if (t[1] > 0) force_cfg = t[1];
      if (t[2] > 0) force_splits = t[2];
    }
  if (L.first) { force_cfg = 2; force_splits = 0; }
  const bool up_ok = cfg_valid(force_cfg) && kTileCfgs[force_cfg].upcat_c == (L.cout % 64 == 0 ? 64 : 32);
  if (L.up && !up_ok) force_cfg = upcat_cfg(L.cout, L.H, L.W);
  return plan_conv(sc, L.n_img, L.H, L.W, L.cin, L.cout, L.partial != nullptr, force_cfg, force_splits, L.up != nullptr,
                   L.pool_out != nullptr);
}

int launch_conv(const ConvLaunch& L, const PlanScope& sc, hipStream_t s, bool* pooled = nullptr) {
  const int cin = L.cin, cout = L.cout, H = L.H, W = L.W;
  const UpSrc* up = L.up;
  if (cin % 32 != 0 || cout % 32 != 0) return PXT_E_ARG;
  if (up && (up->Cp % 32 != 0 || up->Cp >= cin || H != 2 * up->Hp || W != 2 * up->Wp || up->Hs < H || up->Ws < W))
    return PXT_E_ARG;
  const ConvPlan cp = resolve_plan(L, sc);
  const TileCfg& T = kTileCfgs[cp.cfg];
  ConvArgs a;
  a.in = L.in; a.H = H; a.W = W; a.Cin = cin; a.Cout = cout; a.relu = L.relu; a.bias = L.bias;
  a.wpk = cfg_taps(cp.cfg, L.wpk, cin, cout); a.out = L.out; a.partial = L.partial;
  a.up = up ? *up : UpSrc{nullptr, 0, 0, 0, 0, 0};
  a.pool = (cp.splits == 1 && T.pool) ? L.pool_out : nullptr;
  if (T.KS == 2 && ((cin / 32) / cp.splits) % 2 != 0) return PXT_E_ARG;
  if (cp.splits > 1 && (size_t)cp.splits * L.n_img * H * W * cout * sizeof(float) > L.partial_cap) return PXT_E_ARG;
  std::memset(&a.head, 0, sizeof(a.head));
  if (L.head) {
    if (cout != 32 || cp.splits != 1 || cfg_bnc(cp.cfg) != 32) return PXT_E_ARG;
    a.head = *L.head;
    a.head.enabled = 1;
  }
  std::memset(&a.first, 0, sizeof(a.first));
  if (L.first) {
    if (cin != 64 || !T.first || cp.splits != 1 || up) return PXT_E_ARG;
    a.first = *L.first;
    a.first.enabled = 1;
  }
  a.skip.flags = nullptr;
  a.skip.value = nullptr;
  if (L.skip && L.skip->flags && cp.splits == 1 && !L.head && !up && cp.cfg == L.skip_cfg) a.skip = *L.skip;
  if (pooled) *pooled = a.pool != nullptr;
  const dim3 grid(cp.tiles, cp.nb, cp.splits);
  if (knobs().debug)
    fprintf(stderr, "conv layer %2d %4d->%4d @%dx%d x%d  cfg %2d  grid (%d, %d, %d)%s%s\n", sc.layer, cin, cout, W, H, L.n_img,
            cp.cfg, cp.tiles, cp.nb, cp.splits, up ? "  upcat" : "", a.pool ? "  +pool" : "");
  if (launch_tile_cfg(cp.cfg, up != nullptr, sc, a, grid, s) != PXT_OK) return PXT_E_ARG;
  if (cp.splits > 1) {
    const long long n4 = (long long)L.n_img * H * W * cout / 4;
    hipLaunchKernelGGL(splitk_reduce_kernel, dim3((unsigned)((n4 + 255) / 256)), dim3(256), 0, s, L.partial, cp.splits,
                       n4, cout, L.bias, L.relu, L.out);
  }
  return PXT_OK;
}

ConvLaunch pyramid_layer(const pxt_unet* ctx, int li, int H, int W, int n_img) {
  ConvLaunch L;
  L.H = H; L.W = W; L.n_img = n_img; L.cin = ctx->conv[li].cin; L.cout = ctx->conv[li].cout;
  L.wpk = ctx->conv_packed[li]; L.bias = ctx->conv[li].b;
  return L;
}

ConvLaunch encoder_layer(const pxt_unet* ctx, const Plan& P, char* ws, int n_img, int li, const FusedFirst* ff) {
  const int b = enc_block(li);
  ConvLaunch L = pyramid_layer(ctx, li, P.h[b], P.w[b], n_img);
  L.out = (half_t*)(ws + enc_out_offset(P, li));
  L.pool_out = (enc_last(li) && b < 4) ? (half_t*)(ws + P.enc_pool[b + 1]) : nullptr;
  L.first = li == 1 ? ff : nullptr;
  L.partial = L.first ? nullptr : (float*)(ws + P.splitk);
  L.partial_cap = P.splitk_bytes;
  return L;
}

constexpr int kSkipS = 48, kSkipLayers = 6, kSkipMaxC = 256;
int ensure_skip_values(pxt_unet* ctx, const int cfg[kSkipLayers], const PlanScope& scope, hipStream_t s, const half_t** values) {
  ++ctx->skip_clock;
  pxt_unet::SkipEntry* victim = &ctx->skip_cache[0];
  for (auto& e : ctx->skip_cache) {
    if (e.stamp && std::memcmp(e.cfg, cfg, sizeof(e.cfg)) == 0) {
      e.stamp = ctx->skip_clock;
      *values = e.values;
      return PXT_OK;
    }
    if (e.stamp < victim->stamp) victim = &e;
  }
  PXT_HIP_CHECK(hipDeviceSynchronize());
  const size_t raw_b = (size_t)kSkipS * kSkipS * 3 * sizeof(float), map_b = (size_t)kSkipS * kSkipS * kSkipMaxC * sizeof(half_t);
  if (!ctx->skip_scratch) {
    PXT_HIP_CHECK(hipMalloc(&ctx->skip_scratch, raw_b + 2 * map_b));
    PXT_HIP_CHECK(hipMemset(ctx->skip_scratch, 0, raw_b + 2 * map_b));
  }
  if (!victim->values) PXT_HIP_CHECK(hipMalloc((void**)&victim->values, (size_t)kSkipLayers * kSkipMaxC * sizeof(half_t)));
  char* sc = (char*)ctx->skip_scratch;
  half_t* in_map = (half_t*)(sc + raw_b);
// ... 154 lines not shown
extern "C" int pxt_unet_create_f32(const void* weights_host, int64_t n_bytes, pxt_unet** out_ctx) {
  if (!out_ctx) return PXT_E_ARG;
  pxt::UnetF32* net = nullptr;
  const int rc = pxt::f32_create(weights_host, n_bytes, &net);
  if (rc != PXT_OK) return rc;
  pxt_unet* ctx = new pxt_unet();
  ctx->f32 = net;
  *out_ctx = ctx;
  return PXT_OK;
}

extern "C" int pxt_unet_precision(const pxt_unet* ctx) {
  if (!ctx) return PXT_E_ARG;
  return ctx->f32 ? 32 : 16;
}

extern "C" int pxt_unet_destroy(pxt_unet* ctx) {
  if (!ctx) return PXT_E_ARG;
  if (ctx->f32) pxt::f32_destroy(ctx->f32);
  if (ctx->dev_blob) (void)hipFree(ctx->dev_blob);
  if (ctx->dev_head) (void)hipFree(ctx->dev_head);
  if (ctx->dev_packed) (void)hipFree(ctx->dev_packed);
  if (ctx->dev_head0) (void)hipFree(ctx->dev_head0);
  if (ctx->skip_scratch) (void)hipFree(ctx->skip_scratch);
  for (auto& e : ctx->skip_cache)
    if (e.values) (void)hipFree(e.values);
  for (auto& ss : ctx->sides) {
    if (ss.ev_enc4) (void)hipEventDestroy(ss.ev_enc4);
    if (ss.ev_dec1) (void)hipEventDestroy(ss.ev_dec1);
    if (ss.ev_side) (void)hipEventDestroy(ss.ev_side);
  }
  if (ctx->ev_fork) (void)hipEventDestroy(ctx->ev_fork);
  if (ctx->ev_join) (void)hipEventDestroy(ctx->ev_join);
  delete ctx;
  return PXT_OK;
}

extern "C" int64_t pxt_unet_workspace_bytes_batch(const pxt_unet* ctx, int32_t n_images, int32_t H, int32_t W) {
  if (!ctx) return PXT_E_ARG;
  if (ctx->f32) return pxt::f32_workspace_bytes_batch(ctx->f32, n_images, H, W);
  Plan P, P1;
  if (!make_plan(ctx, n_images, H, W, P) || !make_plan(ctx, 1, H, W, P1)) return 0;
  return (int64_t)std::max(P.total, (size_t)n_images * ((P1.total + 255) / 256 * 256));
}

extern "C" int64_t pxt_unet_workspace_bytes(const pxt_unet* ctx, int32_t H, int32_t W) {
  return pxt_unet_workspace_bytes_batch(ctx, 1, H, W);
}

static int forward_pass(pxt_unet* ctx, int32_t n_images, const void* const* images,
                        const int32_t* image_is_u8, const uint8_t* const* masks, int32_t H,
                        int32_t W, float* const* out_maps, const int32_t out_cstride[3],
                        const int32_t* normalize, void* workspace, void* stream, pxt_unet::SideSet& ss,
                        const PlanScope& sc) {
  if (!ctx || !images || !image_is_u8 || !out_maps || !out_cstride || !normalize || !workspace) return PXT_E_ARG;
  Plan P;
  const int B = n_images;
  if (!make_plan(ctx, B, H, W, P)) return PXT_E_ARG;
  for (int i = 0; i < B; ++i) {
    if (!images[i]) return PXT_E_ARG;
    for (int k = 0; k < 3; ++k)
      if (!out_maps[3 * i + k]) return PXT_E_ARG;
  }
  for (int k = 0; k < 3; ++k)
    if (out_cstride[k] < ctx->head[k].cout + 1 || (out_cstride[k] % 4) != 0) return PXT_E_ARG;
  hipStream_t s = (hipStream_t)stream;
  char* ws = (char*)workspace;
  auto buf = [&](size_t off) { return (half_t*)(ws + off); };
  if (!ss.side) {
    ss.side = pxt::shared_side_stream(&ss == &ctx->sides[0] ? 1 : 2);
    if (!ss.side) return PXT_E_HIP;
    PXT_HIP_CHECK(hipEventCreateWithFlags(&ss.ev_enc4, hipEventDisableTiming));
    PXT_HIP_CHECK(hipEventCreateWithFlags(&ss.ev_dec1, hipEventDisableTiming));
    PXT_HIP_CHECK(hipEventCreateWithFlags(&ss.ev_side, hipEventDisableTiming));
  }
  const half_t* pre[5] = {nullptr, nullptr, nullptr, nullptr, nullptr};
  auto head_npix = [&](int k) { return k == 2 ? (long long)P.h[4] * P.w[4] : (long long)P.dh[3 - 2 * k] * P.dw[3 - 2 * k]; };
  auto launch_head = [&](int k, hipStream_t hs) {
    const UnetLayer& Lh = ctx->head[k];
    const long long npix = head_npix(k);
    const long long waves = (npix + 31) / 32;
    const int tpb = waves < 1024 ? 64 : 256;
    const unsigned blocks = (unsigned)((waves * 64 + tpb - 1) / tpb);
    for (int im = 0; im < B; ++im) {
      const half_t* src = pre[2 * k] + (size_t)im * npix * Lh.cin;
      if (Lh.cout + 1 <= 64)
        hipLaunchKernelGGL(head_mfma_kernel<2>, dim3(blocks), dim3(tpb), 0, hs, src, npix, Lh.cin, ctx->head_w[k],
                           ctx->head_b[k], Lh.cout, normalize[im], out_maps[3 * im + k], out_cstride[k]);
      else
        hipLaunchKernelGGL(head_mfma_kernel<5>, dim3(blocks), dim3(tpb), 0, hs, src, npix, Lh.cin, ctx->head_w[k],
                           ctx->head_b[k], Lh.cout, normalize[im], out_maps[3 * im + k], out_cstride[k]);
    }
  };

  const bool merge_heads = knobs().merge_heads && ctx->head[1].cout + 1 > 64 && ctx->head[2].cout + 1 > 64 &&
                           ctx->head[1].cout + 1 <= 160 && ctx->head[2].cout + 1 <= 160;
  auto head_job = [&](int k) {
    const UnetLayer& Lh = ctx->head[k];
    HeadJob j;
    j.in = pre[2 * k]; j.npix = head_npix(k); j.Cin = Lh.cin; j.wts = ctx->head_w[k]; j.bias = ctx->head_b[k];
    j.Cout = Lh.cout; j.normalize = normalize[0]; j.out = out_maps[k]; j.cstride = out_cstride[k];
    j.waves = (j.npix + 31) / 32;
    return j;
  };

  auto fill_images = [&](auto& r) {
    for (int i = 0; i < B; ++i) { r.image[i] = images[i]; r.mask[i] = masks ? masks[i] : nullptr; r.is_u8[i] = image_is_u8[i]; }
// ... 45 lines not shown
          tile_skip[k].value = values + (size_t)k * kSkipMaxC;
        }
      }
    }
  }

  const half_t* skip[5];
  const half_t* cur = nullptr;
  bool pooled_by_conv = false;
  for (int b = 0; b < 5; ++b) {
    const int h = P.h[b], w = P.w[b];
    const half_t* x;
    if (b == 0) {
      const UnetLayer& L0 = ctx->conv[0];
      const unsigned nblk = (unsigned)(((w + kFW - 1) / kFW) * ((h + kFH - 1) / kFH));
      half_t* o = buf(P.enc_tmp[0][0]);
      if (L0.cout != 64) return PXT_E_ARG;
      x = fuse_first ? nullptr : o;
      if (!fuse_first) {
        FirstImages fi;
        fill_images(fi);
        hipLaunchKernelGGL(conv_first_kernel<64>, dim3(nblk, B), dim3(256), 0, s, fi, h, w, (const float*)L0.w, L0.b, o);
      }
    } else {
      half_t* o = buf(P.enc_pool[b]);
      if (!pooled_by_conv) {
        const int cin = ctx->conv[kEnc[b].first].cin;
        const long long n = (long long)B * h * w * (cin / 8);
        hipLaunchKernelGGL(maxpool2_kernel, dim3((unsigned)((n + 255) / 256)), dim3(256), 0, s, cur, P.h[b - 1],
                           P.w[b - 1], cin, o, h, w, B);
      }
      x = o;
    }
    for (int li = std::max(kEnc[b].first, 1); li < kEnc[b].first + kEnc[b].n; ++li) {
      ConvLaunch L = encoder_layer(ctx, P, ws, B, li, fuse_first ? &ff : nullptr);
      L.in = x;
      if (li <= kSkipLayers) { L.skip = &tile_skip[li - 1]; L.skip_cfg = tile_skip_cfg[li - 1]; }
      const int rc = launch_conv(L, sc.at(li), s, &pooled_by_conv);
      if (rc != PXT_OK) return rc;
      x = L.out;
    }
    skip[b] = x;
    cur = x;
  }
  pre[4] = skip[4];
  if (!merge_heads) {
    PXT_HIP_CHECK(hipEventRecord(ss.ev_enc4, s));
    PXT_HIP_CHECK(hipStreamWaitEvent(ss.side, ss.ev_enc4, 0));
    launch_head(2, ss.side);
  }
  const half_t* prev = skip[4];
  bool head0_fused = false;
  int ph = P.h[4], pw = P.w[4], pc = ctx->conv[12].cout;
  for (int d = 0; d < 4; ++d) {
    const UnetLayer& L = ctx->conv[13 + d];
    const int sb = 3 - d;
    const int cs = L.cin - pc;
    if (cs <= 0) return PXT_E_ARG;
    const UpSrc up{prev, ph, pw, pc, P.h[sb], P.w[sb]};
    half_t* o = buf(P.dec_out[d]);
    FusedHead fh;
    const bool fuse_head = d == 3 && ctx->dev_head0 != nullptr && out_cstride[0] >= 36;
    if (fuse_head) {
      const char* hb = (const char*)ctx->dev_head0;
      fh.wfrag = (const half8*)hb;
      fh.conf_w = (const float*)(hb + 2 * 64 * 8 * sizeof(half_t));
      fh.bias = fh.conf_w + 32;
      for (int im = 0; im < B; ++im) { fh.out[im] = out_maps[3 * im]; fh.normalize[im] = normalize[im]; }
      fh.cstride = out_cstride[0];
      fh.enabled = 1;
      head0_fused = true;
    }
    ConvLaunch cl = pyramid_layer(ctx, 13 + d, P.dh[d], P.dw[d], B);
    cl.in = skip[sb]; cl.out = o; cl.up = &up; cl.head = fuse_head ? &fh : nullptr;
    cl.partial = fuse_head ? nullptr : (float*)(ws + P.splitk); cl.partial_cap = P.splitk_bytes;
    const int rc = launch_conv(cl, sc.at(13 + d), s);
    if (rc != PXT_OK) return rc;
    prev = o;
    ph = P.dh[d]; pw = P.dw[d]; pc = L.cout;
    pre[3 - d] = o;
    if (d == 1) {
      PXT_HIP_CHECK(hipEventRecord(ss.ev_dec1, s));
      PXT_HIP_CHECK(hipStreamWaitEvent(ss.side, ss.ev_dec1, 0));
      if (merge_heads && B > 1) {
        HeadBatch hb;
        hb.a = head_job(2);
        hb.b = head_job(1);
        for (int im = 0; im < B; ++im) {
          hb.out_a[im] = out_maps[3 * im + 2];
          hb.out_b[im] = out_maps[3 * im + 1];
          hb.normalize[im] = normalize[im];
        }
        hipLaunchKernelGGL(head_batch_kernel<5>, dim3((unsigned)(hb.a.waves + hb.b.waves), B), dim3(64), 0, ss.side, hb);
      } else if (merge_heads) {
        const HeadJob ja = head_job(2), jb = head_job(1);
        hipLaunchKernelGGL(head_pair_kernel<5>, dim3((unsigned)(ja.waves + jb.waves)), dim3(64), 0, ss.side, ja, jb);
      } else {
        launch_head(1, ss.side);
      }
    }
  }
  if (!head0_fused) launch_head(0, s);
  PXT_HIP_CHECK(hipEventRecord(ss.ev_side, ss.side));
  PXT_HIP_CHECK(hipStreamWaitEvent(s, ss.ev_side, 0));
  PXT_HIP_CHECK(hipGetLastError());
  return PXT_OK;
}

extern "C" int pxt_unet_forward_batch(pxt_unet* ctx, int32_t n_images, const void* const* images,
                                      const int32_t* image_is_u8, const uint8_t* const* masks, int32_t H,
                                      int32_t W, float* const* out_maps, const int32_t out_cstride[3],
                                      const int32_t* normalize, void* workspace, void* stream) {
  if (!ctx || !images || !image_is_u8 || !out_maps || !out_cstride || !normalize || !workspace) return PXT_E_ARG;
  if (ctx->f32)
    return pxt::f32_forward_batch(ctx->f32, n_images, images, image_is_u8, masks, H, W, out_maps, out_cstride, normalize,
                                  workspace, (hipStream_t)stream);
  if (ctx->join_pending) { PXT_HIP_CHECK(hipStreamWaitEvent((hipStream_t)stream, ctx->ev_join, 0)); ctx->join_pending = false; }
  if (n_images != 2 || knobs().streams < 2)
    return forward_pass(ctx, n_images, images, image_is_u8, masks, H, W, out_maps, out_cstride, normalize, workspace,
                        stream, ctx->sides[0], PlanScope{1, ctx->plan_as_single && n_images > 2, 0});
  const int32_t Hs[2] = {H, H}, Ws[2] = {W, W};
  return pxt_unet_forward_pair(ctx, images, image_is_u8, masks, Hs, Ws, out_maps, out_cstride, normalize, workspace, stream);
}

extern "C" int64_t pxt_unet_workspace_bytes_pair(const pxt_unet* ctx, const int32_t H[2], const int32_t W[2]) {
  if (!ctx || !H || !W) return PXT_E_ARG;
  if (ctx->f32) return pxt::f32_workspace_bytes_pair(ctx->f32, H, W);
  Plan P0, P1;
  if (!make_plan(ctx, 1, H[0], W[0], P0) || !make_plan(ctx, 1, H[1], W[1], P1)) return 0;
  return (int64_t)((P0.total + 255) / 256 * 256 + P1.total);
}

extern "C" int pxt_unet_forward_pair(pxt_unet* ctx, const void* const* images, const int32_t* image_is_u8,
                                     const uint8_t* const* masks, const int32_t H[2], const int32_t W[2],
                                     float* const* out_maps, const int32_t out_cstride[3], const int32_t* normalize,
                                     void* workspace, void* stream) {
  if (!ctx || !images || !image_is_u8 || !H || !W || !out_maps || !out_cstride || !normalize || !workspace) return PXT_E_ARG;
  if (ctx->f32)
    return pxt::f32_forward_pair(ctx->f32, images, image_is_u8, masks, H, W, out_maps, out_cstride, normalize, workspace,
                                 (hipStream_t)stream);
  Plan P0, P1;
  if (!make_plan(ctx, 1, H[0], W[0], P0) || !make_plan(ctx, 1, H[1], W[1], P1)) return PXT_E_ARG;
  if (!ctx->pass2) {
    ctx->pass2 = pxt::shared_side_stream(0);
    if (!ctx->pass2) return PXT_E_HIP;
    PXT_HIP_CHECK(hipEventCreateWithFlags(&ctx->ev_fork, hipEventDisableTiming));
    PXT_HIP_CHECK(hipEventCreateWithFlags(&ctx->ev_join, hipEventDisableTiming));
  }
  hipStream_t s = (hipStream_t)stream;
  if (ctx->join_pending) { PXT_HIP_CHECK(hipStreamWaitEvent(s, ctx->ev_join, 0)); ctx->join_pending = false; }
  PXT_HIP_CHECK(hipEventRecord(ctx->ev_fork, s));
  PXT_HIP_CHECK(hipStreamWaitEvent(ctx->pass2, ctx->ev_fork, 0));
  const uint8_t* const no_mask[1] = {nullptr};
  const size_t second = (P0.total + 255) / 256 * 256;
  for (int im = 0; im < 2; ++im) {
    int rc = forward_pass(ctx, 1, images + im, image_is_u8 + im, masks ? masks + im : no_mask, H[im], W[im], out_maps + 3 * im,
                          out_cstride, normalize + im, (char*)workspace + (im ? second : 0),
                          im == 0 ? (void*)s : (void*)ctx->pass2, ctx->sides[im], PlanScope{2, false, 0});
    if (rc != PXT_OK) return rc;
  }
  PXT_HIP_CHECK(hipEventRecord(ctx->ev_join, ctx->pass2));
  if (ctx->defer_join) {
    ctx->join_pending = true;
    return PXT_OK;
  }
  PXT_HIP_CHECK(hipStreamWaitEvent(s, ctx->ev_join, 0));
  return PXT_OK;
}

extern "C" int pxt_unet_set_tile_skip(pxt_unet* ctx, int32_t on) {
  if (!ctx) return PXT_E_ARG;
  ctx->tile_skip = on != 0;
  return PXT_OK;
}

extern "C" int pxt_unet_set_batch_plan(pxt_unet* ctx, int32_t per_image_plan) {
  if (!ctx) return PXT_E_ARG;
  ctx->plan_as_single = per_image_plan != 0;
  return PXT_OK;
}

extern "C" int pxt_unet_set_defer_join(pxt_unet* ctx, int32_t on) {
  if (!ctx) return PXT_E_ARG;
  ctx->defer_join = on != 0;
  return PXT_OK;
}

extern "C" int pxt_unet_pair_join(pxt_unet* ctx, void* stream) {
  if (!ctx) return PXT_E_ARG;
  if (ctx->join_pending) {
    PXT_HIP_CHECK(hipStreamWaitEvent((hipStream_t)stream, ctx->ev_join, 0));
    ctx->join_pending = false;
  }
  return PXT_OK;
}

extern "C" int pxt_unet_forward(pxt_unet* ctx, const void* image, int32_t image_is_u8,
                                const uint8_t* mask, int32_t H, int32_t W, float* const out_maps[3],
                                const int32_t out_cstride[3], int32_t normalize, void* workspace,
                                void* stream) {
  if (!out_maps) return PXT_E_ARG;
  const void* images[1] = {image};
  const uint8_t* masks[1] = {mask};
  return pxt_unet_forward_batch(ctx, 1, images, &image_is_u8, masks, H, W, out_maps, out_cstride, &normalize,
                                workspace, stream);
}

extern "C" int pxt_unet_activation_stats(pxt_unet* ctx, int32_t H, int32_t W, const void* workspace, float* stats,
                                         void* stream) {
  if (!ctx || !workspace || !stats) return PXT_E_ARG;
  if (ctx->f32) return pxt::f32_activation_stats(ctx->f32, H, W, workspace, stats, (hipStream_t)stream);
  Plan P;
  if (!make_plan(ctx, 1, H, W, P)) return PXT_E_ARG;
  hipStream_t s = (hipStream_t)stream;
  if (ctx->join_pending) { PXT_HIP_CHECK(hipStreamWaitEvent(s, ctx->ev_join, 0)); ctx->join_pending = false; }
  PXT_HIP_CHECK(hipMemsetAsync(stats, 0, kNumConv * 2 * sizeof(float), s));
  const char* ws = (const char*)workspace;
  for (int li = 0; li < kNumConv; ++li) {
    const half_t* x = nullptr;
    long long n = 0;
    if (li < kNumEncLayers) {
      const int b = enc_block(li);
      x = (const half_t*)(ws + enc_out_offset(P, li));
      n = (long long)P.h[b] * P.w[b] * ctx->conv[li].cout;
      if (li == 0 && fuses_first(ctx)) x = nullptr;
    } else {
      const int d = li - 13;
      x = (const half_t*)(ws + P.dec_out[d]);
      n = (long long)P.dh[d] * P.dw[d] * ctx->conv[li].cout;
      if (d == 3 && ctx->dev_head0 != nullptr) x = nullptr;
    }
    if (!x) {
      PXT_HIP_CHECK(hipMemsetD32Async((hipDeviceptr_t)(stats + 2 * li), 0xBF800000u, 1, s));
      continue;
    }
    hipLaunchKernelGGL(activation_stats_kernel, dim3(512), dim3(256), 0, s, x, n / 8, stats + 2 * li);
  }
  PXT_HIP_CHECK(hipGetLastError());
  return PXT_OK;
}

extern "C" int64_t pxt_conv3x3_packed_bytes(int32_t Cin, int32_t Cout) {
  if (Cin < 32 || Cout < 32 || Cin % 32 != 0 || Cout % 32 != 0) return PXT_E_ARG;
  return (int64_t)2 * Cout * 9 * Cin * (int64_t)sizeof(half_t);
}

extern "C" int pxt_conv3x3_pack_weights(const void* weights, int32_t Cin, int32_t Cout, void* packed, void* stream) {
  if (!weights || !packed || pxt_conv3x3_packed_bytes(Cin, Cout) <= 0) return PXT_E_ARG;
  const long long n = (long long)Cout * 9 * Cin;
  hipLaunchKernelGGL(pack_conv_weights_kernel, dim3((unsigned)((n + 255) / 256)), dim3(256), 0, (hipStream_t)stream,
                     (const half_t*)weights, Cin, Cout, (half_t*)packed);
  hipLaunchKernelGGL(pack_conv_weights_v3_kernel, dim3((unsigned)((n + 255) / 256)), dim3(256), 0, (hipStream_t)stream,
                     (const half_t*)weights, Cin, Cout, (half_t*)packed + n);
  PXT_HIP_CHECK(hipGetLastError());
  return PXT_OK;
}

extern "C" int pxt_conv3x3_packed(const void* in, int32_t H, int32_t W, int32_t Cin, const void* packed,
// ... 44 lines not shown
```

pixtrack_amd/feature_extractor.py:

```python
from __future__ import annotations

from typing import Dict, Optional, Tuple

import numpy as np
import torch

from . import _lib
from .ops import ops
from .unet import OUTPUT_DIMS
from .utils.conf import merge


class PixTrackFeatureExtractor:
    default_conf: Dict = dict(resize=1024, resize_by="max")

    def __init__(self, model, device: torch.device, conf: Optional[Dict] = None):
        self.conf = merge(self.default_conf, conf or {})
        self.device = torch.device(device)
        self.model = model
        self._staged = None
        self._ready = None
        import os

        self.defer_join = os.environ.get("PXT_UNET_DEFER_JOIN", "1") != "0" and hasattr(model, "set_defer_join")
# ... 17 lines not shown
        return h, w, scale_resize

    def _to_device_hwc(self, image) -> torch.Tensor:
        if isinstance(image, np.ndarray):
            image = torch.from_numpy(np.ascontiguousarray(image))
        if image.dtype not in (torch.float32, torch.uint8):
            image = image.float()
        return image.to(self.device, non_blocking=True).contiguous()

    def stage(self, image, scale_image: int = 1, mask: Optional[torch.Tensor] = None,
              normalize: bool = False) -> None:
        self._join()
        self._staged = (image, scale_image, mask, normalize)
        self._ready = None

    def preload(self, image, scale_image: int, mask, normalize: bool, maps, scales) -> None:
        self._preloaded.append((image, scale_image, mask, normalize, maps, scales))

    def prepared(self, image, scale_image: int = 1, mask=None):
        a_img, a_mask, a_sr = self._prepare(image, scale_image, mask)
        return a_img, a_mask, [(a_sr[0] / s, a_sr[1] / s) for s in self.model.scales]

    def unstage(self) -> None:
        self._join()
        self._staged = self._ready = None
        self._preloaded.clear()

    def _join(self) -> None:
        if self._join_pending:
            self.model.join()
            self._join_pending = False

    def _prepare(self, image, scale_image, mask):
        img = self._to_device_hwc(image)
        H, W = int(img.shape[0]), int(img.shape[1])
        h_new, w_new, scale_resize = self.target_size(H, W, scale_image)
        if (h_new, w_new) != (H, W):
            active = None
            if mask is not None:
                mask = mask.to(self.device, torch.uint8).contiguous()
                active = torch.empty(h_new, w_new, dtype=torch.uint8, device=self.device)
                ops.resize_activity(mask, None, H, W, active)
                img = img.float() * mask[..., None].float()
            elif img.dtype == torch.uint8:
                active = torch.empty(h_new, w_new, dtype=torch.uint8, device=self.device)
                ops.resize_activity(None, img, H, W, active)
            mask = active
            src = img.float().contiguous()
            dst = torch.empty(h_new, w_new, 3, device=self.device, dtype=torch.float32)
            ops.resize_linear(src, dst)
            img = dst
        return img, mask, scale_resize

    def extract_packed(self, image, scale_image: int = 1, mask: Optional[torch.Tensor] = None,
                       normalize: bool = False):
        for k, r in enumerate(self._preloaded):
            if r[0] is image and r[1] == scale_image and r[2] is mask and r[3] == normalize:
                del self._preloaded[k]
                self.last_input_wh = (int(r[4][0].shape[1]), int(r[4][0].shape[0]))
                return r[4], r[5]
        if self._ready is not None:
            r = self._ready
            self._ready = None
            self._join()
            if r[0] is image and r[1] == scale_image and r[2] is mask and r[3] == normalize:
                return r[4], r[5]
        a_img, a_mask, a_sr = self._prepare(image, scale_image, mask)
        self.last_input_wh = (int(a_img.shape[1]), int(a_img.shape[0]))
        scales = [(a_sr[0] / s, a_sr[1] / s) for s in self.model.scales]
        if self._staged is not None:
            st_image, st_scale, st_mask, st_norm = self._staged
            self._staged = None
            if st_image is not image:
                b_img, b_mask, b_sr = self._prepare(st_image, st_scale, st_mask)
                if self.defer_join:
                    self.model.set_defer_join(True)
                try:
                    both = self.model.forward_packed_batch([(a_img, a_mask, normalize), (b_img, b_mask, st_norm)])
                finally:
                    if self.defer_join:
                        self.model.set_defer_join(False)
                        self._join_pending = True
                self._ready = (st_image, st_scale, st_mask, st_norm, both[1],
                               [(b_sr[0] / s, b_sr[1] / s) for s in self.model.scales], b_img, b_mask)
                return both[0], scales
        return self.model.forward_packed(a_img, a_mask, normalize=normalize), scales

    @torch.no_grad()
    def __call__(self, image: np.ndarray, scale_image: int = 1):
        maps, scales = self.extract_packed(image, scale_image, None, normalize=False)
        features = [m[..., :c].permute(2, 0, 1) for m, c in zip(maps, OUTPUT_DIMS)]
        confidences = [m[..., c : c + 1].permute(2, 0, 1) for m, c in zip(maps, OUTPUT_DIMS)]
        assert len(self.model.scales) == len(features)
        return features, scales, confidences
```

pixtrack_amd/ops.py:

```python
from __future__ import annotations

import ctypes as C
from typing import List, Optional, Sequence

import torch

from . import _lib

_NS = "pixtrack"
_DEF = torch.library.Library(_NS, "DEF")

SCHEMAS = {
    "lm_refine": (
        "(Tensor p3d, Tensor? point_mask, Tensor[] fmaps, Tensor[] frefs, int[] channels, float[] cameras, "
        "int[] ndist, float[] lambdas, float[] T_init, int num_iters, int pad, int loss, float loss_alpha, "
        "float loss_scale, float grad_stop, float dt_stop, float dR_stop, int min_valid, int n_workgroups, "
        "Tensor(a!) record, Tensor(b!) workspace, bool want_log, int spin_limit=0, float[]? cam_conv=None, "
        "int[]? cam_slots=None, Tensor(c!)? cam_out=None, int lm_path=0) -> ()"),
    "lm_refine_batch": (
        "(Tensor[] p3d, Tensor?[] point_masks, int[] n_levels, Tensor[] fmaps, Tensor[] frefs, int[] channels, "
        "float[] cameras, int[] ndist, float[] lambdas, float[] T_init, int num_iters, int pad, int loss, float loss_alpha, "
        "float loss_scale, float grad_stop, float dt_stop, float dR_stop, int min_valid, int n_workgroups, "
        "Tensor(a!)[] records, Tensor(b!)[] workspaces, Tensor(c!) batch_workspace, bool want_log, int spin_limit=0, "
        "float[]? cam_conv=None, int[]? cam_slots=None, Tensor(d!)[]? cam_outs=None, int lm_path=0, "
        "int[]? cam_enabled=None) -> ()"),
    "lm_information": (
        "(Tensor[] p3d, Tensor?[] point_masks, Tensor[] fmaps, Tensor[] frefs, int[] channels, float[] cameras, "
        "int[] ndist, Tensor[] poses, bool pose_is_lm_record, int pad, int loss, float loss_alpha, float loss_scale, "
        "int min_valid, Tensor(a!)[] records, Tensor(b!) workspace) -> ()"),
    "lm_point_report": (
        "(Tensor[] p3d, Tensor?[] point_masks, Tensor[] fmaps, Tensor[] frefs, int[] channels, float[] cameras, "
        "int[] ndist, Tensor[] poses, bool pose_is_lm_record, int pad, int loss, float loss_alpha, float loss_scale, "
        "int min_valid, float[] inlier_weights, Tensor(a!)?[] points, Tensor(b!)[] summaries, Tensor(c!) workspace) -> ()"),
    "sample_sparse": (
        "(Tensor p3d, float[] T, Tensor[] fmaps, int[] channels, float[] cameras, int[] ndist, int pad, "
        "bool normalize, Tensor(a!)[] outs, Tensor(b!) valid, int[]? windows=None) -> ()"),
    "score_pose_hypotheses": (
        "(Tensor fmap, int channels, float[] camera, int ndist, Tensor p3d, Tensor fref, Tensor? valid, Tensor poses, "
        "Tensor ranges, int pad, int loss, float loss_alpha, float loss_scale, Tensor(a!) out) -> ()"),
    "unet_forward_batch": (
        "(int ctx, Tensor[] images, Tensor?[] masks, bool[] normalize, Tensor(a!)[] outs, Tensor(b!) workspace) -> ()"),
    "ngp_render": (
        "(int ctx, float[] view, int width, int height, int spp, int mode, Tensor(a!) out, Tensor(b!)? stats) -> ()"),
    "ngp_render_both": (
        "(int ctx, float[] view, int width, int height, int spp, Tensor(a!) rgba, Tensor(b!) depth, "
        "Tensor(c!)? stats) -> ()"),
    "ngp_render_both_from_pose": (
        "(int ctx, float[] view, Tensor pose_record, float[] conv, int width, int height, int spp, int mode, "
        "Tensor(a!) rgba, Tensor(b!)? depth, Tensor(c!) cam_out, Tensor(d!)? stats) -> ()"),
    "ngp_render_frame": (
        "(int ctx, float[] view, int width, int height, int spp, int mode, bool camera_from_slot, Tensor(a!)? rgba, "
        "Tensor(b!)? depth, Tensor(c!)? rgb_u8, Tensor(d!)? depth_nz, Tensor(e!)? stats) -> ()"),
    "ngp_render_frame_batch": (
        "(int[] ctxs, float[] views, int[] sizes, int spp, int[] modes, bool camera_from_slot, Tensor(a!)[] rgb_u8, "
        "Tensor(b!)[] depth_nz, Tensor(c!) workspace, Tensor(d!)[] stats, Tensor(e!)[]? depth_float=None) -> ()"),
    "depth_mask": "(Tensor depth_rgba, int n_erode, int n_dilate, Tensor(a!) mask, Tensor(b!) scratch) -> ()",
    "depth_mask_plane": "(Tensor depth_nz, int n_erode, int n_dilate, Tensor(a!) mask) -> ()",
    "rgba_to_u8": "(Tensor rgba, float alpha_thresh, Tensor(a!) out) -> ()",
    "resize_linear": "(Tensor src, Tensor(a!) dst) -> ()",
    "resize_activity": "(Tensor? mask, Tensor? image_u8, int H, int W, Tensor(a!) active) -> ()",
    "conv3x3_nhwc_f16": "(Tensor x, Tensor weight, Tensor bias, bool relu, Tensor(a!) out) -> ()",
    "points_from_depth": (
        "(Tensor depth, float[] xform, float focal, float depth_scale, float min_alpha, int erode, int n_max, "
        "Tensor(a!) p3d, Tensor(b!) slot_valid, Tensor(c!) record, Tensor(d!) workspace) -> ()"),
    "pose_errors": (
        "(Tensor vertices, Tensor rel_poses, bool want_adds, Tensor(a!) records, Tensor(b!) workspace) -> ()"),
    "depth_agreement": (
        "(Tensor depth_est, Tensor depth_gt, float min_alpha, float[] tq, Tensor(a!) records, "
        "Tensor(b!) workspace) -> ()"),
    "symmetric_pose_errors": (
        "(Tensor vertices, Tensor syms, Tensor frames, Tensor(a!) records, Tensor(b!) workspace) -> ()"),
    "sensor_vsd": (
        "(Tensor depth_est, Tensor depth_gt, Tensor sensor, Tensor? ray, int[] shift, float min_alpha, float sensor_q, "
        "float delta_q, float[] tq, Tensor(a!) records, Tensor(b!) workspace) -> ()"),
}
for _name, _schema in SCHEMAS.items():
    _DEF.define(_name + _schema)

VIEW_FLOATS = 12 + 2 + 3 + 3 + 4 + 1


def _stream(t: torch.Tensor) -> int:
    return int(torch.cuda.current_stream(t.device).cuda_stream)


def _f32c(t: torch.Tensor, what: str) -> torch.Tensor:
    if t.dtype != torch.float32 or not t.is_contiguous():
        raise _lib.PxtError(f"{what} must be a contiguous float32 tensor (got {t.dtype}, contiguous={t.is_contiguous()})")
    return t


def _lm_refine(p3d, point_mask, fmaps, frefs, channels, cameras, ndist, lambdas, T_init, num_iters, pad, loss,
               loss_alpha, loss_scale, grad_stop, dt_stop, dR_stop, min_valid, n_workgroups, record, workspace,
               want_log, spin_limit=0, cam_conv=None, cam_slots=None, cam_out=None, lm_path=0):
# ... 242 lines not shown
        arr[i].ndist = int(ndist[i])
        if windows is not None:
            arr[i].x0, arr[i].y0, arr[i].full_w, arr[i].full_h = (int(x) for x in windows[4 * i:4 * i + 4])
    if valid.dtype != torch.uint8 or valid.numel() != n:
        raise _lib.PxtError("sample_sparse: valid must be uint8 [n_points]")
    T12 = (C.c_float * 12)(*[float(x) for x in T])
    _lib.check(L.pxt_sample_sparse(p3d.data_ptr(), n, T12, arr, n_levels, int(pad), int(bool(normalize)),
                                   valid.data_ptr(), _stream(p3d)), "pxt_sample_sparse")


def _score_pose_hypotheses(fmap, channels, camera, ndist, p3d, fref, valid, poses, ranges, pad, loss, loss_alpha, loss_scale,
                           out):
    L = _lib.lib()
    _f32c(fmap, "fmap")
    _f32c(p3d, "p3d")
    _f32c(fref, "fref")
    _f32c(poses, "poses")
    _f32c(out, "out")
    if fmap.dim() != 3 or len(camera) != 10:
        raise _lib.PxtError("score_pose_hypotheses: fmap is [h, w, cstride], camera 10 floats")
    h, w, cs = (int(x) for x in fmap.shape)
    n = int(p3d.shape[0])
    if tuple(p3d.shape) != (n, 3) or tuple(fref.shape) != (n, cs):
        raise _lib.PxtError(f"score_pose_hypotheses: p3d {tuple(p3d.shape)} / fref {tuple(fref.shape)}, expected "
                            f"{(n, 3)} / {(n, cs)}")
    if valid is not None and (valid.dtype != torch.uint8 or not valid.is_contiguous() or valid.numel() != n):
        raise _lib.PxtError("score_pose_hypotheses: valid must be contiguous uint8 [n_points]")
    M = int(poses.shape[0]) if poses.dim() == 2 else -1
    if M < 1 or tuple(poses.shape) != (M, 12):
        raise _lib.PxtError(f"score_pose_hypotheses: poses is {tuple(poses.shape)}, expected [M >= 1, 12]")
    if ranges.dtype != torch.int32 or not ranges.is_contiguous() or tuple(ranges.shape) != (M, 2):
        raise _lib.PxtError("score_pose_hypotheses: ranges must be contiguous int32 [M, 2]")
    if out.numel() != 4 * M:
        raise _lib.PxtError("score_pose_hypotheses: out holds 4 floats per hypothesis")
    for t, name in ((fmap, "fmap"), (p3d, "p3d"), (fref, "fref"), (valid, "valid"), (poses, "poses"), (ranges, "ranges"),
                    (out, "out")):
        if t is None:
            continue
        _lib.require_gpu(t, name)
        if t.device != fmap.device:
            raise _lib.PxtError(f"score_pose_hypotheses: {name} is on {t.device}, the map on {fmap.device}")
    mp = _lib.RelocMap()
    mp.fmap, mp.h, mp.w, mp.C, mp.cstride = fmap.data_ptr(), h, w, int(channels), cs
    mp.cam[:] = [float(x) for x in camera]
    mp.ndist = int(ndist)
    bank = _lib.RelocBank()
    bank.p3d, bank.fref, bank.valid, bank.n_points = p3d.data_ptr(), fref.data_ptr(), _lib.dptr(valid), n
    conf = _lib.LmConf()
    conf.pad, conf.loss, conf.loss_alpha, conf.loss_scale = int(pad), int(loss), float(loss_alpha), float(loss_scale)
    _lib.check(L.pxt_score_pose_hypotheses(C.byref(mp), C.byref(bank), poses.data_ptr(), ranges.data_ptr(), M, C.byref(conf),
                                           out.data_ptr(), _stream(fmap)), "pxt_score_pose_hypotheses")


def _unet_forward_batch(ctx, images, masks, normalize, outs, workspace):
    L = _lib.lib()
    n = len(images)
    if n == 0 or len(masks) != n or len(normalize) != n or len(outs) != 3 * n:
        raise _lib.PxtError("unet_forward_batch: per image one mask slot, one normalize flag and three output maps")
    sizes = [(int(im.shape[0]), int(im.shape[1])) for im in images]
    H, W = sizes[0]
    pair = n == 2 and sizes[1] != sizes[0]
    for im, mk, hw in zip(images, masks, sizes):
        if im.dim() != 3 or im.shape[2] != 3 or not im.is_contiguous() or im.dtype not in (torch.float32, torch.uint8):
            raise _lib.PxtError("unet_forward_batch: images are contiguous HWC, 3 channels, float32 or uint8")
        if hw != (H, W) and not pair:
            raise _lib.PxtError("unet_forward_batch: a batch of more than two holds images of one size")
        if mk is not None and (mk.dtype != torch.uint8 or tuple(mk.shape) != hw or not mk.is_contiguous()):
            raise _lib.PxtError("unet_forward_batch: masks are contiguous uint8 [H, W]")
    Hs = (C.c_int32 * 2)(sizes[0][0], sizes[-1][0])
    Ws = (C.c_int32 * 2)(sizes[0][1], sizes[-1][1])
    need = int(L.pxt_unet_workspace_bytes_pair(ctx, Hs, Ws)) if pair else int(L.pxt_unet_workspace_bytes_batch(ctx, n, H, W))
    if need <= 0:
        raise _lib.PxtError(f"images {sizes} are not supported by the 4-level encoder")
    if workspace.numel() * workspace.element_size() < need:
        raise _lib.PxtError(f"unet_forward_batch: workspace holds {workspace.numel()} bytes, {need} needed")
    for o in outs:
        _f32c(o, "out map")
    imgs = (C.c_void_p * n)(*[im.data_ptr() for im in images])
    is_u8 = (C.c_int32 * n)(*[int(im.dtype == torch.uint8) for im in images])
    mks = (C.c_void_p * n)(*[_lib.dptr(m) for m in masks])
    norm = (C.c_int32 * n)(*[int(bool(x)) for x in normalize])
    ptrs = (C.c_void_p * (3 * n))(*[o.data_ptr() for o in outs])
    cs = (C.c_int32 * 3)(*[int(o.shape[2]) for o in outs[:3]])
    if pair:
        _lib.check(L.pxt_unet_forward_pair(ctx, imgs, is_u8, mks, Hs, Ws, ptrs, cs, norm, workspace.data_ptr(),
                                           _stream(images[0])), "pxt_unet_forward_pair")
    else:
        _lib.check(L.pxt_unet_forward_batch(ctx, n, imgs, is_u8, mks, H, W, ptrs, cs, norm, workspace.data_ptr(),
                                            _stream(images[0])), "pxt_unet_forward_batch")


def _conv3x3(x, weight, bias, relu, out):
    H, W, Cin = (int(s) for s in x.shape)
    Cout = int(weight.shape[0])
    _lib.check(_lib.lib().pxt_conv3x3_nhwc_f16(x.data_ptr(), H, W, Cin, weight.data_ptr(), bias.data_ptr(), Cout,
                                               int(bool(relu)), out.data_ptr(), _stream(x)), "pxt_conv3x3_nhwc_f16")


def _view(view: Sequence[float], width, height, spp, mode) -> "_lib.NgpView":
    if len(view) != VIEW_FLOATS:
        raise _lib.PxtError(f"ngp view record has {len(view)} floats, expected {VIEW_FLOATS}")
    v = _lib.NgpView()
    v.cam[:] = view[0:12]
    v.focal, v.k1 = view[12], view[13]
    v.aabb_min[:] = view[14:17]
    v.aabb_max[:] = view[17:20]
    v.background[:] = view[20:24]
    v.min_transmittance = view[24]
    v.width, v.height, v.spp, v.mode = int(width), int(height), int(spp), int(mode)
    return v


def _check_frame(t: torch.Tensor, width, height, what):
    _f32c(t, what)
    if tuple(t.shape) != (height, width, 4):
        raise _lib.PxtError(f"{what} must be [{height}, {width}, 4] (got {tuple(t.shape)})")


def _ngp_render(ctx, view, width, height, spp, mode, out, stats):
    _check_frame(out, width, height, "out")
    v = _view(view, width, height, spp, mode)
    _lib.check(_lib.lib().pxt_ngp_render(ctx, C.byref(v), out.data_ptr(), _lib.dptr(stats), _stream(out)),
               "pxt_ngp_render")


def _ngp_render_both(ctx, view, width, height, spp, rgba, depth, stats):
    _check_frame(rgba, width, height, "rgba")
    _check_frame(depth, width, height, "depth")
    v = _view(view, width, height, spp, 0)
    _lib.check(_lib.lib().pxt_ngp_render_both(ctx, C.byref(v), rgba.data_ptr(), depth.data_ptr(), _lib.dptr(stats),
                                              _stream(rgba)), "pxt_ngp_render_both")


def _ngp_render_both_from_pose(ctx, view, pose_record, conv, width, height, spp, mode, rgba, depth, cam_out, stats):
    _check_frame(rgba, width, height, "rgba")
    if depth is not None:
        _check_frame(depth, width, height, "depth")
# ... 338 lines not shown
```

pixtrack_amd/refiner.py:

```python
from __future__ import annotations

import ctypes as C
import logging
from typing import Dict, List, Optional, Sequence, Tuple

import math

import numpy as np
import torch

from . import _lib
from .ops import ops
from .feature_extractor import PixTrackFeatureExtractor
from .geometry import Camera, Pose
from .model3d import Model3D
from .optimizer import LevelPack, PixTrackOptimizer, cstride_for
from .unet import OUTPUT_DIMS, UNet
from .utils.conf import Conf, merge

logger = logging.getLogger(__name__)
import os as _os

_WINDOW_ENV = _os.environ.get("PXT_REF_WINDOW", "1") != "0"

# ... 131 lines not shown
    WINDOW_MIN_SAVING = 0.35

    def reference_window(self, dbids, pose: Optional[Pose], reference_image):
        memo = self.__dict__.get("_window_memo")
        if memo is not None and memo[0] is reference_image and memo[1] is pose:
            return memo[2], memo[3]
        out = (reference_image, None)
        if self.conf.get("reference_window", True) and _WINDOW_ENV and torch.is_tensor(reference_image) and pose is not None \
                and (self.conf.multiscale or [1]) == [1]:
            H, W = int(reference_image.shape[0]), int(reference_image.shape[1])
            ex = self.feature_extractor
            if ex.target_size(H, W, 1)[:2] == (H, W):
                self._points_of(dbids)
                xyz = self._p3d_host[int(dbids[0])]
                image = self.model3d.dbs[dbids[0]]
                cam = self._reference_camera_of(image.camera_id)
                R, t = pose.numpy()
                p = xyz @ np.asarray(R, np.float64).T + np.asarray(t, np.float64)
                front = p[:, 2] > 1e-3
                if front.any():
                    c10 = [float(x) for x in cam.as10().tolist()]
                    fx, fy, cx, cy, k1, k2, p1, p2 = c10[2:10]
                    xn, yn = p[front, 0] / p[front, 2], p[front, 1] / p[front, 2]
                    r2 = xn * xn + yn * yn
                    rad = k1 * r2 + k2 * r2 * r2
                    xd = xn + xn * rad + 2.0 * p1 * xn * yn + p2 * (r2 + 2.0 * xn * xn)
                    yd = yn + yn * rad + 2.0 * p2 * xn * yn + p1 * (r2 + 2.0 * yn * yn)
                    u, v = fx * xd + cx, fy * yd + cy
                    inside = (u >= 0) & (v >= 0) & (u <= W - 1) & (v <= H - 1)
                    if inside.any():
                        m = self.WINDOW_MARGIN
                        x0 = max(0, int(np.floor(u[inside].min()) - m) // 16 * 16)
                        y0 = max(0, int(np.floor(v[inside].min()) - m) // 16 * 16)
                        x1 = min(W, -(-(int(np.ceil(u[inside].max())) + 1 + m) // 16) * 16)
                        y1 = min(H, -(-(int(np.ceil(v[inside].max())) + 1 + m) // 16) * 16)
                        if (x1 - x0) * (y1 - y0) <= (1.0 - self.WINDOW_MIN_SAVING) * W * H and x1 - x0 >= 64 and y1 - y0 >= 64 \
                                and ex.target_size(y1 - y0, x1 - x0, 1)[:2] == (y1 - y0, x1 - x0):
                            out = (reference_image[y0:y1, x0:x1].contiguous(), (x0, y0, W, H))
        self._window_memo = (reference_image, pose, out[0], out[1])
        return out

    def _reference_camera_of(self, camera_id) -> Camera:
        ck = (camera_id, float(self.reference_scale))
        cams_memo = self.__dict__.setdefault("_ref_cameras", {})
        camera = cams_memo.get(ck)
        if camera is None:
            camera = cams_memo[ck] = Camera.from_colmap(self.model3d.cameras[camera_id]).scale(self.reference_scale)
        return camera

    def warm_reference_points(self, dbids: Optional[Sequence[int]] = None) -> None:
        for dbid in (dbids if dbids is not None else list(self.model3d.dbs)):
            self._points_of([int(dbid)])

    def dense_feature_extraction(self, image, name: str, image_scale: int = 1, mask=None, normalize=False):
        maps, scales = self.feature_extractor.extract_packed(image, image_scale, mask, normalize)
        if self.tracker is not None and getattr(self.tracker, "debug", 0) >= 2:
            feats = [m[..., :c].permute(2, 0, 1) for m, c in zip(maps, OUTPUT_DIMS)]
            weight = [m[..., c : c + 1].permute(2, 0, 1) for m, c in zip(maps, OUTPUT_DIMS)]
            self.log_dense(name=name, image=image, image_scale=image_scale, features=feats, scales=scales,
                           weight=weight)
        return maps, scales

    def interp_sparse_observations(self, feature_maps: List[torch.Tensor], feature_scales, image_id: int,
                                   p3dids: List[int], pose: Optional[Pose] = None,
                                   p3d: Optional[torch.Tensor] = None, window=None) -> SparseReferenceFeatures:
        image = self.model3d.dbs[image_id]
        camera = self._reference_camera_of(image.camera_id)
        T_w2cam = Pose.from_colmap(image) if pose is None else pose
        if p3d is None:
            p3d = torch.from_numpy(np.array([self.model3d.points3D[p].xyz for p in p3dids], np.float32)).to(self.device)
        n = int(p3d.shape[0])
        outs, cams, ndist = [], [], []
        for fm, sc in zip(feature_maps, feature_scales):
            outs.append(torch.empty(n, fm.shape[2], device=self.device, dtype=torch.float32))
            cam_l = camera.scale(sc)
            cams += cam_l.as10().tolist()
            ndist.append(int(cam_l._data.shape[-1] - 6))
        valid = torch.empty(n, dtype=torch.uint8, device=self.device)
        pad = self.optimizer[0].interpolator.pad
        T12 = T_w2cam.as12().detach().cpu().reshape(-1).tolist()
        windows = None
        if window is not None:
            x0, y0, fw, fh = window
            windows = []
            for fm, stride in zip(feature_maps, self.feature_extractor.model.scales):
                lh, lw = self.feature_extractor.model.level_shapes(fh, fw)[len(windows) // 4]
                windows += [x0 // stride, y0 // stride, lw, lh]
        ops.sample_sparse(p3d, T12, list(feature_maps), list(OUTPUT_DIMS[:len(feature_maps)]), cams, ndist, int(pad),
                          True, outs, valid, windows)
        return SparseReferenceFeatures(outs, valid, list(p3dids), p3d, OUTPUT_DIMS)

    def extract_reference_features(self, dbids, pose: Optional[Pose] = None, reference_image=None, depth=None,
                                   depth_view=None):
        multiscales = self.conf.multiscale or [1]
        if reference_image is None:
            raise NotImplementedError("static reference images on disk (r5/r7 mode) are out of scope: "
                                      "r9 always passes the NeRF render (pixloc_tracker_r9.py:157-159)")
        ref_img = self.model3d.dbs[dbids[0]]
        if pose is None:
            pose = Pose.from_Rt(ref_img.qvec2rotmat(), ref_img.tvec)
        render_points = self.render_points
        if render_points:
            if depth is None or depth_view is None:
                raise ValueError("reference_points='render' needs the frame's Depth render (depth, depth_view)")
            p3d, slot_valid, record = self.points_from_render(depth, depth_view)
            p3dids = self.__dict__.get("_slot_ids")
            if p3dids is None or len(p3dids) != int(p3d.shape[0]):
                p3dids = self._slot_ids = list(range(int(p3d.shape[0])))
        else:
            p3dids, p3d = self._points_of(dbids)
        features = {}
        for image_scale in multiscales:
            image, window = (reference_image, None) if render_points else self.reference_window(dbids, pose, reference_image)
            maps, scales = self.dense_feature_extraction(image, ref_img.name, image_scale)
            self.last_reference_wh = self.feature_extractor.last_input_wh
            features[str(image_scale)] = self.interp_sparse_observations(maps, scales, dbids[0], p3dids, pose, p3d, window)
            if render_points:
                features[str(image_scale)].slot_valid, features[str(image_scale)].points_record = slot_valid, record
            else:
                features[str(image_scale)].p3d_host = self._p3d_host[int(dbids[0])]
        return features

    def _feature_cache_paths(self):
        from pathlib import Path

        dumps = Path(self.paths.get("dumps", "."))
        return dumps / "reference_features.h5", dumps / "reference_features.npz"

    def read_features(self, ref_id) -> Dict[str, SparseReferenceFeatures]:
        h5_path, npz_path = self._feature_cache_paths()
        multiscales = self.conf.multiscale or [1]
        arrays = {}
        if h5_path.exists():
            try:
                import h5py
            except ImportError as e:
                raise _lib.PxtError(f"{h5_path} needs h5py, which this environment lacks; convert it to "
                                    f"{npz_path.name} (same keys, '/'-joined)") from e
            with h5py.File(str(h5_path), "r") as f:
                for scale in multiscales:
                    g = f[str(ref_id)][str(scale)]
                    arrays[f"{scale}/p3dids"] = np.array(g["p3dids"])
                    for level in (k for k in g.keys() if k != "p3dids"):
                        arrays[f"{scale}/{level}/p3did_to_feat"] = np.array(g[level]["p3did_to_feat"])
        elif npz_path.exists():
            with np.load(npz_path) as z:
                pre = f"{ref_id}/"
                arrays = {k[len(pre):]: z[k] for k in z.files if k.startswith(pre)}
        else:
            raise FileNotFoundError(f"no reference feature cache at {h5_path} or {npz_path}")
        out = {}
        for scale in multiscales:
            p3dids = [int(x) for x in arrays[f"{scale}/p3dids"].tolist()]
            packed = []
            for level, c in enumerate(OUTPUT_DIMS):
                feat = torch.from_numpy(np.asarray(arrays[f"{scale}/{level}/p3did_to_feat"], np.float32))
                assert feat.shape == (len(p3dids), c + 1), (feat.shape, len(p3dids), c)
                rec = torch.zeros(len(p3dids), cstride_for(c))
                d = feat[:, :c]
                rec[:, :c] = d / d.norm(dim=1, keepdim=True).clamp_min(1e-12)
                rec[:, c] = feat[:, c]
                packed.append(rec.to(self.device))
            xyz = np.array([self.model3d.points3D[p].xyz for p in p3dids], np.float32).reshape(-1, 3)
            valid = torch.ones(len(p3dids), dtype=torch.uint8, device=self.device)
            out[str(scale)] = SparseReferenceFeatures(packed, valid, p3dids, torch.from_numpy(xyz).to(self.device),
                                                      OUTPUT_DIMS)
        return out
# ... 277 lines not shown
```

pixtrack_amd/unet.py:

```python
from __future__ import annotations

import ctypes as C
import struct
from typing import Dict, List, Optional, Tuple

import numpy as np
import torch

from . import _lib
from .ops import ops
from .optimizer import cstride_for

ENC_BLOCKS = [[(3, 64), (64, 64)], [(64, 128), (128, 128)], [(128, 256), (256, 256), (256, 256)],
              [(256, 512), (512, 512), (512, 512)], [(512, 512), (512, 512), (512, 512)]]
SKIP_DIMS = [64, 128, 256, 512, 512]
DECODER = [64, 64, 64, 32]
OUTPUT_SCALES = [0, 2, 4]
OUTPUT_DIMS = [32, 128, 128]
HEAD_INPUTS = [32, 64, 512]
BN_EPS = 1e-5
MAGIC = b"PXTUNET1"
MAGIC_F32 = b"PXTUNF32"
PRECISIONS = ("fp16", "fp32")

# ... 220 lines not shown


class UNet:

    scales = [1, 4, 16]
    output_dims = OUTPUT_DIMS

    def __init__(self, weights: Dict[str, torch.Tensor], device: torch.device, precision: str = "fp16"):
        self.device = torch.device(device)
        if self.device.type != "cuda":
            raise _lib.PxtError("UNet needs a ROCm device; no CPU path exists")
        if precision not in PRECISIONS:
            raise _lib.PxtError(f"UNet precision must be one of {PRECISIONS}, got {precision!r}")
        self.precision = precision
        blob = pack_unet_weights(weights, precision)
        import hashlib

        self.weights_signature = f"{precision}:{hashlib.sha1(blob).hexdigest()}"
        self._ctx = C.c_void_p()
        create = "pxt_unet_create" if precision == "fp16" else "pxt_unet_create_f32"
        with torch.cuda.device(self.device):
            _lib.check(getattr(_lib.lib(), create)(blob, len(blob), C.byref(self._ctx)), create)
        self._ws: Optional[torch.Tensor] = None

    def __del__(self):
        try:
            if getattr(self, "_ctx", None):
                _lib.lib().pxt_unet_destroy(self._ctx)
                self._ctx = None
        except Exception:
            pass

    def eval(self):
        return self

    def to(self, device):
        assert torch.device(device) == self.device
        return self

    @staticmethod
    def level_shapes(H: int, W: int) -> List[Tuple[int, int]]:
        hs, ws = [H], [W]
        for _ in range(4):
            hs.append(hs[-1] // 2)
            ws.append(ws[-1] // 2)
        dh, dw = hs[4], ws[4]
        dec = []
        for _ in range(4):
            dh, dw = dh * 2, dw * 2
            dec.append((dh, dw))
        return [dec[3], dec[1], (hs[4], ws[4])]

    def forward_packed(self, image: torch.Tensor, mask: Optional[torch.Tensor] = None,
                       normalize: bool = False) -> List[torch.Tensor]:
        return self.forward_packed_batch([(image, mask, normalize)])[0]

    def forward_packed_batch(self, items) -> List[List[torch.Tensor]]:
        n = len(items)
        sizes = [(int(it[0].shape[0]), int(it[0].shape[1])) for it in items]
        H, W = sizes[0]
        for image, _mask, _ in items:
            _lib.require_gpu(image, "image")
        if n == 2 and sizes[1] != sizes[0]:
            Hs, Ws = (C.c_int32 * 2)(sizes[0][0], sizes[1][0]), (C.c_int32 * 2)(sizes[0][1], sizes[1][1])
            need = int(_lib.lib().pxt_unet_workspace_bytes_pair(self._ctx, Hs, Ws))
        else:
            need = int(_lib.lib().pxt_unet_workspace_bytes_batch(self._ctx, n, H, W))
        if need <= 0:
            raise _lib.PxtError(f"images {sizes} are not supported by the 4-level encoder")
        if self._ws is None or self._ws.numel() < need:
            self._ws = torch.empty(need, dtype=torch.uint8, device=self.device)
        outs = [[torch.empty(h, w, cstride_for(c), device=self.device, dtype=torch.float32)
                 for (h, w), c in zip(self.level_shapes(*hw), OUTPUT_DIMS)] for hw in sizes]
        ops.unet_forward_batch(int(self._ctx.value), [it[0] for it in items], [it[1] for it in items],
                               [bool(it[2]) for it in items], [o for per in outs for o in per], self._ws)
        return outs

    def set_batch_plan(self, per_image_plan: bool) -> None:
        _lib.check(_lib.lib().pxt_unet_set_batch_plan(self._ctx, int(bool(per_image_plan))), "pxt_unet_set_batch_plan")

    def set_tile_skip(self, on: bool) -> None:
        _lib.check(_lib.lib().pxt_unet_set_tile_skip(self._ctx, int(bool(on))), "pxt_unet_set_tile_skip")

    def set_defer_join(self, on: bool) -> None:
        _lib.check(_lib.lib().pxt_unet_set_defer_join(self._ctx, int(bool(on))), "pxt_unet_set_defer_join")

    def join(self) -> None:
        _lib.check(_lib.lib().pxt_unet_pair_join(self._ctx, _lib.stream_ptr(self.device)), "pxt_unet_pair_join")

    def activation_stats(self, image: torch.Tensor, mask: Optional[torch.Tensor] = None):
        self.forward_packed(image, mask, normalize=False)
        H, W = int(image.shape[0]), int(image.shape[1])
        stats = torch.zeros(34, dtype=torch.float32, device=self.device)
        _lib.check(_lib.lib().pxt_unet_activation_stats(self._ctx, H, W, self._ws.data_ptr(), stats.data_ptr(),
                                                        _lib.stream_ptr(self.device)), "pxt_unet_activation_stats")
        h = stats.cpu()
        counts = h.view(torch.int32)
        return [None if float(h[2 * l]) < 0 else (float(h[2 * l]), int(counts[2 * l + 1])) for l in range(17)]

    def __call__(self, data: Dict[str, torch.Tensor]) -> Dict[str, List[torch.Tensor]]:
        image = data["image"]
        assert image.dim() == 4 and image.shape[0] == 1 and image.shape[1] == 3
        hwc = (image[0].permute(1, 2, 0) * 255.0).to(self.device, torch.float32).contiguous()
        outs = self.forward_packed(hwc, None, normalize=False)
        feats = [o[..., :c].permute(2, 0, 1)[None] for o, c in zip(outs, OUTPUT_DIMS)]
        confs = [o[..., c : c + 1].permute(2, 0, 1)[None] for o, c in zip(outs, OUTPUT_DIMS)]
        return {"feature_maps": feats, "confidences": confs}
```

Before: 742.0.

## Skip decoder tiles not touched by reference point samples in UNet

When extracting reference-image features, the 3D points are projected on the device to mark which fine-level decoder tiles (and the upsample source tiles they read) are actually sampled by the later sparse interpolation. Decoder convolutions for unmarked tiles then return early, without computing or filling outputs. This cuts UNet decoder work for reference frames, at the cost of an extra small marking kernel and leaving unsampled regions of the feature maps uninitialized.

```diff
diff --git a/include/pixtrack_hip.h b/include/pixtrack_hip.h
--- a/include/pixtrack_hip.h
+++ b/include/pixtrack_hip.h
@@ -171,6 +171,27 @@
                           const uint8_t* const* masks, const int32_t H[2], const int32_t W[2],
                           float* const* out_maps, const int32_t out_cstride[3], const int32_t* normalize,
                           void* workspace, void* stream);
+typedef struct {
+  const float* p3d;
+  int32_t n_points;
+  float T[12];
+  float cam[10];
+  int32_t ndist, pad;
+  int32_t x0, y0, full_w, full_h;
+} pxt_unet_sample_points;
+int pxt_unet_forward_sampled(pxt_unet* ctx, const void* image, int32_t image_is_u8, const uint8_t* mask, int32_t H,
+                             int32_t W, float* const out_maps[3], const int32_t out_cstride[3], int32_t normalize,
+                             void* workspace, void* stream, const pxt_unet_sample_points* points_host);
+int pxt_unet_forward_pair_sampled(pxt_unet* ctx, const void* const* images, const int32_t* image_is_u8,
+                                  const uint8_t* const* masks, const int32_t H[2], const int32_t W[2],
+                                  float* const* out_maps, const int32_t out_cstride[3], const int32_t* normalize,
+                                  void* workspace, void* stream,
+                                  const pxt_unet_sample_points* const* points_host );
+int pxt_unet_set_reference_tiles(pxt_unet* ctx, int32_t on);
+int pxt_unet_reference_tiles_host(const pxt_unet_sample_points* points_host, int32_t fine_h, int32_t fine_w,
+                                  int32_t fine_tile_rows, int32_t low_tile_rows, uint8_t* fine_flags_host,
+                                  uint8_t* low_flags_host);
+
 int pxt_unet_set_defer_join(pxt_unet* ctx, int32_t on);
 int pxt_unet_pair_join(pxt_unet* ctx, void* stream);
 
diff --git a/pixtrack_amd/_lib.py b/pixtrack_amd/_lib.py
--- a/pixtrack_amd/_lib.py
+++ b/pixtrack_amd/_lib.py
@@ -84,6 +84,21 @@
     ]
 
 
+class UnetSamplePoints(C.Structure):
+    _fields_ = [
+        ("p3d", C.c_void_p),
+        ("n_points", C.c_int32),
+        ("T", C.c_float * 12),
+        ("cam", C.c_float * 10),
+        ("ndist", C.c_int32),
+        ("pad", C.c_int32),
+        ("x0", C.c_int32),
+        ("y0", C.c_int32),
+        ("full_w", C.c_int32),
+        ("full_h", C.c_int32),
+    ]
+
+
 class NgpModel(C.Structure):
     _fields_ = [
         ("n_levels", C.c_int32),
@@ -190,6 +205,17 @@
         C.c_int,
         [_VP, _VP, _I32, _VP, _I32, _I32, C.POINTER(_VP), C.POINTER(_I32), _I32, _VP, _VP],
     ),
+    "pxt_unet_forward_sampled": (
+        C.c_int,
+        [_VP, _VP, _I32, _VP, _I32, _I32, C.POINTER(_VP), C.POINTER(_I32), _I32, _VP, _VP, C.POINTER(UnetSamplePoints)],
+    ),
+    "pxt_unet_forward_pair_sampled": (
+        C.c_int,
+        [_VP, C.POINTER(_VP), C.POINTER(_I32), C.POINTER(_VP), C.POINTER(_I32), C.POINTER(_I32), C.POINTER(_VP),
+         C.POINTER(_I32), C.POINTER(_I32), _VP, _VP, C.POINTER(C.POINTER(UnetSamplePoints))],
+    ),
+    "pxt_unet_set_reference_tiles": (C.c_int, [_VP, _I32]),
+    "pxt_unet_reference_tiles_host": (C.c_int, [C.POINTER(UnetSamplePoints), _I32, _I32, _I32, _I32, _VP, _VP]),
     "pxt_unet_set_defer_join": (C.c_int, [_VP, _I32]),
     "pxt_unet_set_batch_plan": (C.c_int, [_VP, _I32]),
     "pxt_unet_set_tile_skip": (C.c_int, [_VP, _I32]),
diff --git a/pixtrack_amd/csrc/pxt_common.h b/pixtrack_amd/csrc/pxt_common.h
--- a/pixtrack_amd/csrc/pxt_common.h
+++ b/pixtrack_amd/csrc/pxt_common.h
@@ -35,7 +35,7 @@
 
 constexpr float kCamEps = 1e-3f;
 
-__device__ inline bool project_point(const Cam& c, float x, float y, float z, float& u, float& v,
+__host__ __device__ inline bool project_point(const Cam& c, float x, float y, float z, float& u, float& v,
                                      float* J ) {
   bool visible = z > kCamEps;
   float zc = fmaxf(z, kCamEps);
diff --git a/pixtrack_amd/csrc/pxt_conv_v2.h b/pixtrack_amd/csrc/pxt_conv_v2.h
--- a/pixtrack_amd/csrc/pxt_conv_v2.h
+++ b/pixtrack_amd/csrc/pxt_conv_v2.h
@@ -50,6 +50,10 @@
     }
   }
 }
+
+constexpr int kUpPatchW = 10;
+__host__ __device__ constexpr int up_patch_rows(int TH) { return TH / 2 + 2; }
+__host__ __device__ constexpr int up_patch_origin(int t0) { return (t0 >> 1) - 1; }
 
 struct ConvArgs {
   const half_t* in;
@@ -151,6 +155,7 @@
   const half_t* in = a.in + (size_t)img * (UPCAT ? a.up.Hs : H) * in_w * Cs;
   const half_t* prev = UPCAT ? a.up.prev + (size_t)img * a.up.Hp * a.up.Wp * a.up.Cp : nullptr;
   if (a.skip.flags != nullptr && a.skip.flags[blockIdx.x] == 0) {
+    if (a.skip.value == nullptr) return;
     conv_fill_constant_tile<TH, BNC, 256>(a.skip.value, a.out + (size_t)img * H * W * Cout,
                                           a.pool ? a.pool + (size_t)img * (H >> 1) * (W >> 1) * Cout : nullptr, H, W, Cout, ty0,
                                           tx0, co0);
@@ -220,13 +225,13 @@
     }
   };
 
-  constexpr int PH = TH / 2 + 2, PW = 10;
+  constexpr int PH = up_patch_rows(TH), PW = kUpPatchW;
   constexpr int kPatchElems = PH * PW * 4, KP = (kPatchElems + 255) / 256;
   static_assert(!UPCAT || KP <= KB, "the patch pieces reuse the halo staging registers");
   char* const patch = smem + 2 * kBuf;
   unsigned poff[UPCAT ? KP : 1], up_src[UPCAT ? KH : 1];
   if (UPCAT) {
-    const int py0 = (ty0 >> 1) - 1, px0 = (tx0 >> 1) - 1;
+    const int py0 = up_patch_origin(ty0), px0 = up_patch_origin(tx0);
 #pragma unroll
     for (int kp = 0; kp < KP; ++kp) {
       const int i = min(tid + 256 * kp, kPatchElems - 1);
diff --git a/pixtrack_amd/csrc/pxt_conv_v3.h b/pixtrack_amd/csrc/pxt_conv_v3.h
--- a/pixtrack_amd/csrc/pxt_conv_v3.h
+++ b/pixtrack_amd/csrc/pxt_conv_v3.h
@@ -80,6 +80,7 @@
   const half_t* in = a.in + (size_t)img * (UPCAT ? a.up.Hs : H) * in_w * Cs;
   const half_t* prev = UPCAT ? a.up.prev + (size_t)img * a.up.Hp * a.up.Wp * a.up.Cp : nullptr;
   if (a.skip.flags != nullptr && a.skip.flags[blockIdx.x] == 0) {
+    if (a.skip.value == nullptr) return;
     conv_fill_constant_tile<TH, BNC, 256 * KS>(a.skip.value, a.out + (size_t)img * H * W * Cout,
                                                a.pool ? a.pool + (size_t)img * (H >> 1) * (W >> 1) * Cout : nullptr, H, W, Cout,
                                                ty0, tx0, co0);
@@ -154,12 +155,12 @@
     if (i < kElems) *(half8*)(s_halo + buf * kBuf + hy * G::kRow + hx * G::kPix + ((seg ^ G::swz(hx)) << 4)) = r_in[k];
   };
 
-  constexpr int PH = TH / 2 + 2, PW = 10;
+  constexpr int PH = up_patch_rows(TH), PW = kUpPatchW;
   constexpr int kPatchElems = PH * PW * G::kNP, KP = (kPatchElems + 255) / 256;
   static_assert(!UPCAT || KP <= KH, "the patch pieces reuse the halo staging registers");
   unsigned poff[UPCAT ? KP : 1], up_src[UPCAT ? KH : 1];
   if constexpr (UPCAT) {
-    const int py0 = (ty0 >> 1) - 1, px0 = (tx0 >> 1) - 1;
+    const int py0 = up_patch_origin(ty0), px0 = up_patch_origin(tx0);
 #pragma unroll
     for (int kp = 0; kp < KP; ++kp) {
       const int i = min(tid + 256 * kp, kPatchElems - 1);
diff --git a/pixtrack_amd/csrc/pxt_lm.hip b/pixtrack_amd/csrc/pxt_lm.hip
--- a/pixtrack_amd/csrc/pxt_lm.hip
+++ b/pixtrack_amd/csrc/pxt_lm.hip
@@ -732,15 +732,11 @@
     for (int c0 = 4 * sub; c0 < cs; c0 += 4 * LG) *(float4*)(o + c0) = make_float4(0, 0, 0, 0);
     return false;
   }
-  const float fu = floorf(u), fv = floorf(v);
-  const int ix0f = (int)fu, iy0f = (int)fv;
-  const float ax = u - fu, ay = v - fv;
-  const int x1f = min(ix0f + 1, FW - 1), y1f = min(iy0f + 1, FH - 1);
-  const float mx = (ix0f + 1 < FW) ? 1.f : 0.f, my = (iy0f + 1 < FH) ? 1.f : 0.f;
+  const SampleTexels tx = sample_texels(u, v, FW, FH, L.x0, L.y0, W, H);
+  const float ax = tx.ax, ay = tx.ay, mx = tx.mx, my = tx.my;
   const float w00 = (1.f - ax) * (1.f - ay), w10 = ax * (1.f - ay) * mx, w01 = (1.f - ax) * ay * my,
               w11 = ax * ay * mx * my;
-  const int ix0 = min(max(ix0f - L.x0, 0), W - 1), iy0 = min(max(iy0f - L.y0, 0), H - 1);
-  const int x1 = min(max(x1f - L.x0, 0), W - 1), y1 = min(max(y1f - L.y0, 0), H - 1);
+  const int ix0 = tx.ix0, iy0 = tx.iy0, x1 = tx.x1, y1 = tx.y1;
   const float* p00 = L.fmap + ((size_t)iy0 * W + ix0) * cs;
   const float* p10 = L.fmap + ((size_t)iy0 * W + x1) * cs;
   const float* p01 = L.fmap + ((size_t)y1 * W + ix0) * cs;
diff --git a/pixtrack_amd/csrc/pxt_lm_point.h b/pixtrack_amd/csrc/pxt_lm_point.h
--- a/pixtrack_amd/csrc/pxt_lm_point.h
+++ b/pixtrack_amd/csrc/pxt_lm_point.h
@@ -79,13 +79,13 @@
   return lm_dpp_add(v, 3);
 }
 
-__device__ inline void transform_point(const float* T, float X, float Y, float Z, float& px, float& py, float& pz) {
+__host__ __device__ inline void transform_point(const float* T, float X, float Y, float Z, float& px, float& py, float& pz) {
   px = T[0] * X + T[1] * Y + T[2] * Z + T[9];
   py = T[3] * X + T[4] * Y + T[5] * Z + T[10];
   pz = T[6] * X + T[7] * Y + T[8] * Z + T[11];
 }
 
-__device__ inline void point_in_window(const Cam& cam, float px, float py, float pz, bool& valid, int W, int H, float pad,
+__host__ __device__ inline void point_in_window(const Cam& cam, float px, float py, float pz, bool& valid, int W, int H, float pad,
                                        float& u, float& v, float* Jw ) {
   valid = project_point(cam, px, py, pz, u, v, Jw) && valid;
   valid = valid && (u >= pad) && (v >= pad) && (u <= (float)(W - 1) - pad) && (v <= (float)(H - 1) - pad);
@@ -101,6 +101,27 @@
   w10 = ax * (1.f - ay);
   w01 = (1.f - ax) * ay;
   w11 = ax * ay;
+}
+
+struct SampleTexels {
+  int ix0, iy0, x1, y1;
+  float ax, ay, mx, my;
+};
+__host__ __device__ inline int clamp_int(int v, int lo, int hi) { return v < lo ? lo : (v > hi ? hi : v); }
+__host__ __device__ inline SampleTexels sample_texels(float u, float v, int FW, int FH, int x0, int y0, int W, int H) {
+  SampleTexels t;
+  const float fu = floorf(u), fv = floorf(v);
+  const int ix0f = (int)fu, iy0f = (int)fv;
+  t.ax = u - fu;
+  t.ay = v - fv;
+  const int x1f = ix0f + 1 < FW ? ix0f + 1 : FW - 1, y1f = iy0f + 1 < FH ? iy0f + 1 : FH - 1;
+  t.mx = (ix0f + 1 < FW) ? 1.f : 0.f;
+  t.my = (iy0f + 1 < FH) ? 1.f : 0.f;
+  t.ix0 = clamp_int(ix0f - x0, 0, W - 1);
+  t.iy0 = clamp_int(iy0f - y0, 0, H - 1);
+  t.x1 = clamp_int(x1f - x0, 0, W - 1);
+  t.y1 = clamp_int(y1f - y0, 0, H - 1);
+  return t;
 }
 
 #define PXT_LM_POINT_CH(w00_, w10_, w01_, w11_, a01_, a02_, a10_, a11_, a12_, a13_, a20_, a21_, a22_, a23_, a31_, a32_, \
diff --git a/pixtrack_amd/csrc/pxt_unet.hip b/pixtrack_amd/csrc/pxt_unet.hip
--- a/pixtrack_amd/csrc/pxt_unet.hip
+++ b/pixtrack_amd/csrc/pxt_unet.hip
@@ -1,4 +1,5 @@
 #include "pxt_common.h"
+#include "pxt_lm_point.h"
 #include "pxt_unet_f32.h"
 
 #include <algorithm>
@@ -387,6 +388,54 @@
   if (i < C) dst[i] = src[i];
 }
 
+struct RefPoints {
+  const float* p3d;
+  int n;
+  float T[12], cam[10];
+  int ndist;
+  float pad;
+  int x0, y0, fw, fh;
+  int W, H;
+};
+struct RefTileGeo {
+  int th, tiles_x, tiles_y;
+};
+__host__ __device__ inline void reference_tiles_mark(const RefPoints& P, int n, const RefTileGeo& fine, uint8_t* fine_flags) {
+  const Cam cam = make_cam(P.cam, P.ndist);
+  float px, py, pz, u = 0.f, v = 0.f;
+  transform_point(P.T, P.p3d[3 * n], P.p3d[3 * n + 1], P.p3d[3 * n + 2], px, py, pz);
+  bool valid = true;
+  point_in_window(cam, px, py, pz, valid, P.fw, P.fh, P.pad, u, v, nullptr);
+  if (!valid) return;
+  const SampleTexels t = sample_texels(u, v, P.fw, P.fh, P.x0, P.y0, P.W, P.H);
+  const int c0 = t.ix0 >> 4, c1 = t.x1 >> 4, r0 = t.iy0 / fine.th, r1 = t.y1 / fine.th;
+  fine_flags[r0 * fine.tiles_x + c0] = 1;
+  fine_flags[r0 * fine.tiles_x + c1] = 1;
+  fine_flags[r1 * fine.tiles_x + c0] = 1;
+  fine_flags[r1 * fine.tiles_x + c1] = 1;
+}
+__host__ __device__ inline void reference_tiles_spread(int i, const RefTileGeo& fine, const uint8_t* fine_flags,
+                                                       const RefTileGeo& low, int low_h, int low_w, uint8_t* low_flags) {
+  if (!fine_flags[i]) return;
+  const int ty0 = (i / fine.tiles_x) * fine.th, tx0 = (i % fine.tiles_x) * 16;
+  const int py0 = up_patch_origin(ty0), px0 = up_patch_origin(tx0);
+  const int ya = clamp_int(py0, 0, low_h - 1), yb = clamp_int(py0 + up_patch_rows(fine.th) - 1, 0, low_h - 1);
+  const int xa = clamp_int(px0, 0, low_w - 1), xb = clamp_int(px0 + kUpPatchW - 1, 0, low_w - 1);
+  for (int r = ya / low.th; r <= yb / low.th; ++r)
+    for (int c = xa >> 4; c <= (xb >> 4); ++c) low_flags[r * low.tiles_x + c] = 1;
+}
+__global__ __launch_bounds__(1024) void reference_tiles_kernel(const RefPoints P, const RefTileGeo fine, const RefTileGeo low,
+                                                               int low_h, int low_w, uint8_t* __restrict__ fine_flags,
+                                                               uint8_t* __restrict__ low_flags) {
+  const int n_fine = fine.tiles_x * fine.tiles_y, n_low = low.tiles_x * low.tiles_y;
+  for (int i = threadIdx.x; i < n_fine; i += blockDim.x) fine_flags[i] = 0;
+  for (int i = threadIdx.x; i < n_low; i += blockDim.x) low_flags[i] = 0;
+  __syncthreads();
+  for (int n = threadIdx.x; n < P.n; n += blockDim.x) reference_tiles_mark(P, n, fine, fine_flags);
+  __syncthreads();
+  for (int i = threadIdx.x; i < n_fine; i += blockDim.x) reference_tiles_spread(i, fine, fine_flags, low, low_h, low_w, low_flags);
+}
+
 struct UnetLayer {
   int cin, cout;
   const void* w;
@@ -418,6 +467,7 @@
   } skip_cache[8];
   unsigned long long skip_clock = 0;
   bool tile_skip = true;
+  bool ref_tiles = true;
   void* skip_scratch = nullptr;
   bool plan_as_single = false;
   bool defer_join = false;
@@ -439,11 +489,13 @@
   }
   return v;
 }
+constexpr int kRefTilesDefault = 1;
 struct Knobs {
   int streams = env_int("PXT_UNET_STREAMS", 2);
   bool merge_heads = env_int("PXT_UNET_MERGE_HEADS", 1) != 0;
   bool skip = env_int("PXT_UNET_SKIP", 1) != 0;
   bool fuse_first = env_int("PXT_UNET_FUSE_FIRST", 1) != 0;
+  bool ref_tiles = env_int("PXT_UNET_REF_TILES", kRefTilesDefault) != 0;
   const char* plan_env = getenv("PXT_CONV_PLAN");
   std::vector<std::array<int, 3>> plan = parse_plan(plan_env);
   bool debug = getenv("PXT_CONV_DEBUG") != nullptr;
@@ -564,6 +616,7 @@
   int dh[4], dw[4];
   size_t enc_tmp[5][2], enc_pool[5], enc_out[5], dec_out[4], splitk, splitk_bytes, total;
   size_t skip_grid, skip_flags;
+  size_t ref_flags, ref_flags_each;
   int skip_bh, skip_bw;
 };
 
@@ -600,6 +653,8 @@
   P.skip_bw = (W + 7) / 8;
   P.skip_grid = take((size_t)n_img * P.skip_bh * P.skip_bw);
   P.skip_flags = take((size_t)n_img * 6 * ((size_t)(H / 8 + 2) * (W / 16 + 2)));
+  P.ref_flags_each = align256((size_t)(H / 8 + 2) * (W / 16 + 2));
+  P.ref_flags = take(2 * P.ref_flags_each);
   P.total = off;
   return true;
 }
@@ -667,6 +722,8 @@
   const FusedHead* head = nullptr;
   const FusedFirst* first = nullptr;
   const TileSkip* skip = nullptr;
+  const uint8_t* needed = nullptr;
+  int needed_cfg = 0;
 };
 
 ConvPlan resolve_plan(const ConvLaunch& L, const PlanScope& sc) {
@@ -713,6 +770,7 @@
   a.skip.flags = nullptr;
   a.skip.value = nullptr;
   if (L.skip && L.skip->flags && cp.splits == 1 && !L.head && !up && cp.cfg == L.skip_cfg) a.skip = *L.skip;
+  if (L.needed && !a.skip.flags && cp.splits == 1 && L.n_img == 1 && cp.cfg == L.needed_cfg) a.skip.flags = L.needed;
   if (pooled) *pooled = a.pool != nullptr;
   const dim3 grid(cp.tiles, cp.nb, cp.splits);
   if (knobs().debug)
@@ -973,7 +1031,7 @@
                         const int32_t* image_is_u8, const uint8_t* const* masks, int32_t H,
                         int32_t W, float* const* out_maps, const int32_t out_cstride[3],
                         const int32_t* normalize, void* workspace, void* stream, pxt_unet::SideSet& ss,
-                        const PlanScope& sc) {
+                        const PlanScope& sc, const pxt_unet_sample_points* pts = nullptr) {
   if (!ctx || !images || !image_is_u8 || !out_maps || !out_cstride || !normalize || !workspace) return PXT_E_ARG;
   Plan P;
   const int B = n_images;
@@ -1125,6 +1183,52 @@
   const half_t* prev = skip[4];
   bool head0_fused = false;
   int ph = P.h[4], pw = P.w[4], pc = ctx->conv[12].cout;
+  const bool fuse_head3 = ctx->dev_head0 != nullptr && out_cstride[0] >= 36;
+  auto decoder_layer = [&](int d, const UpSrc* up) {
+    ConvLaunch cl = pyramid_layer(ctx, 13 + d, P.dh[d], P.dw[d], B);
+    cl.up = up;
+    cl.partial = (d == 3 && fuse_head3) ? nullptr : (float*)(ws + P.splitk);
+    cl.partial_cap = P.splitk_bytes;
+    return cl;
+  };
+  const uint8_t* ref_needed[2] = {nullptr, nullptr};
+  int ref_cfg[2] = {0, 0};
+  if (pts && pts->p3d && B == 1 && knobs().ref_tiles && ctx->ref_tiles && fuse_head3) {
+    const int FW = P.dw[3], FH = P.dh[3];
+    const bool windowed = pts->full_w > 0;
+    if (pts->n_points < 0 || pts->pad < 0 ||
+        (windowed && (pts->full_h < 1 || pts->x0 < 0 || pts->y0 < 0 || pts->x0 + FW > pts->full_w || pts->y0 + FH > pts->full_h)))
+      return PXT_E_ARG;
+    const UpSrc planned{prev, 1, 1, 32, 1, 1};
+    RefTileGeo geo[2];
+    bool ok = true;
+    for (int k = 0; k < 2; ++k) {
+      const ConvPlan cp = resolve_plan(decoder_layer(2 + k, &planned), sc.at(15 + k));
+      ok = ok && cfg_valid(cp.cfg);
+      if (!ok) break;
+      ref_cfg[k] = cp.cfg;
+      geo[k].th = cfg_th(cp.cfg);
+      geo[k].tiles_x = (P.dw[2 + k] + 15) / 16;
+      geo[k].tiles_y = (P.dh[2 + k] + geo[k].th - 1) / geo[k].th;
+      ok = ok && (size_t)geo[k].tiles_x * geo[k].tiles_y <= P.ref_flags_each;
+    }
+    if (ok) {
+      RefPoints rp;
+      rp.p3d = pts->p3d; rp.n = pts->n_points;
+      for (int i = 0; i < 12; ++i) rp.T[i] = pts->T[i];
+      for (int i = 0; i < 10; ++i) rp.cam[i] = pts->cam[i];
+      rp.ndist = pts->ndist; rp.pad = (float)pts->pad;
+      rp.x0 = windowed ? pts->x0 : 0; rp.y0 = windowed ? pts->y0 : 0;
+      rp.fw = windowed ? pts->full_w : FW; rp.fh = windowed ? pts->full_h : FH;
+      rp.W = FW; rp.H = FH;
+      uint8_t* fine_flags = (uint8_t*)(ws + P.ref_flags);
+      uint8_t* low_flags = fine_flags + P.ref_flags_each;
+      hipLaunchKernelGGL(reference_tiles_kernel, dim3(1), dim3(1024), 0, s, rp, geo[1], geo[0], P.dh[2], P.dw[2], fine_flags,
+                         low_flags);
+      ref_needed[0] = low_flags;
+      ref_needed[1] = fine_flags;
+    }
+  }
   for (int d = 0; d < 4; ++d) {
     const UnetLayer& L = ctx->conv[13 + d];
     const int sb = 3 - d;
@@ -1133,7 +1237,7 @@
     const UpSrc up{prev, ph, pw, pc, P.h[sb], P.w[sb]};
     half_t* o = buf(P.dec_out[d]);
     FusedHead fh;
-    const bool fuse_head = d == 3 && ctx->dev_head0 != nullptr && out_cstride[0] >= 36;
+    const bool fuse_head = d == 3 && fuse_head3;
     if (fuse_head) {
       const char* hb = (const char*)ctx->dev_head0;
       fh.wfrag = (const half8*)hb;
@@ -1144,9 +1248,9 @@
       fh.enabled = 1;
       head0_fused = true;
     }
-    ConvLaunch cl = pyramid_layer(ctx, 13 + d, P.dh[d], P.dw[d], B);
-    cl.in = skip[sb]; cl.out = o; cl.up = &up; cl.head = fuse_head ? &fh : nullptr;
-    cl.partial = fuse_head ? nullptr : (float*)(ws + P.splitk); cl.partial_cap = P.splitk_bytes;
+    ConvLaunch cl = decoder_layer(d, &up);
+    cl.in = skip[sb]; cl.out = o; cl.head = fuse_head ? &fh : nullptr;
+    if (d >= 2) { cl.needed = ref_needed[d - 2]; cl.needed_cfg = ref_cfg[d - 2]; }
     const int rc = launch_conv(cl, sc.at(13 + d), s);
     if (rc != PXT_OK) return rc;
     prev = o;
@@ -1204,14 +1308,18 @@
   return (int64_t)((P0.total + 255) / 256 * 256 + P1.total);
 }
 
-extern "C" int pxt_unet_forward_pair(pxt_unet* ctx, const void* const* images, const int32_t* image_is_u8,
-                                     const uint8_t* const* masks, const int32_t H[2], const int32_t W[2],
-                                     float* const* out_maps, const int32_t out_cstride[3], const int32_t* normalize,
-                                     void* workspace, void* stream) {
+extern "C" int pxt_unet_forward_pair_sampled(pxt_unet* ctx, const void* const* images, const int32_t* image_is_u8,
+                                             const uint8_t* const* masks, const int32_t H[2], const int32_t W[2],
+                                             float* const* out_maps, const int32_t out_cstride[3], const int32_t* normalize,
+                                             void* workspace, void* stream,
+                                             const pxt_unet_sample_points* const* points_host) {
   if (!ctx || !images || !image_is_u8 || !H || !W || !out_maps || !out_cstride || !normalize || !workspace) return PXT_E_ARG;
   if (ctx->f32)
     return pxt::f32_forward_pair(ctx->f32, images, image_is_u8, masks, H, W, out_maps, out_cstride, normalize, workspace,
                                  (hipStream_t)stream);
+  if (points_host && knobs().streams < 2 && H[0] == H[1] && W[0] == W[1])
+    return pxt_unet_forward_batch(ctx, 2, images, image_is_u8, masks, H[0], W[0], out_maps, out_cstride, normalize, workspace,
+                                  stream);
   Plan P0, P1;
   if (!make_plan(ctx, 1, H[0], W[0], P0) || !make_plan(ctx, 1, H[1], W[1], P1)) return PXT_E_ARG;
   if (!ctx->pass2) {
@@ -1229,7 +1337,8 @@
   for (int im = 0; im < 2; ++im) {
     int rc = forward_pass(ctx, 1, images + im, image_is_u8 + im, masks ? masks + im : no_mask, H[im], W[im], out_maps + 3 * im,
                           out_cstride, normalize + im, (char*)workspace + (im ? second : 0),
-                          im == 0 ? (void*)s : (void*)ctx->pass2, ctx->sides[im], PlanScope{2, false, 0});
+                          im == 0 ? (void*)s : (void*)ctx->pass2, ctx->sides[im], PlanScope{2, false, 0},
+                          points_host ? points_host[im] : nullptr);
     if (rc != PXT_OK) return rc;
   }
   PXT_HIP_CHECK(hipEventRecord(ctx->ev_join, ctx->pass2));
@@ -1238,6 +1347,49 @@
     return PXT_OK;
   }
   PXT_HIP_CHECK(hipStreamWaitEvent(s, ctx->ev_join, 0));
+  return PXT_OK;
+}
+
+extern "C" int pxt_unet_forward_pair(pxt_unet* ctx, const void* const* images, const int32_t* image_is_u8,
+                                     const uint8_t* const* masks, const int32_t H[2], const int32_t W[2],
+                                     float* const* out_maps, const int32_t out_cstride[3], const int32_t* normalize,
+                                     void* workspace, void* stream) {
+  return pxt_unet_forward_pair_sampled(ctx, images, image_is_u8, masks, H, W, out_maps, out_cstride, normalize, workspace,
+                                       stream, nullptr);
+}
+
+extern "C" int pxt_unet_set_reference_tiles(pxt_unet* ctx, int32_t on) {
+  if (!ctx) return PXT_E_ARG;
+  ctx->ref_tiles = on != 0;
+  return PXT_OK;
+}
+
+extern "C" int pxt_unet_reference_tiles_host(const pxt_unet_sample_points* points_host, int32_t fine_h, int32_t fine_w,
+                                             int32_t fine_tile_rows, int32_t low_tile_rows, uint8_t* fine_flags_host,
+                                             uint8_t* low_flags_host) {
+  const pxt_unet_sample_points* pts = points_host;
+  if (!pts || (!pts->p3d && pts->n_points > 0) || pts->n_points < 0 || pts->pad < 0 || !fine_flags_host || !low_flags_host)
+    return PXT_E_ARG;
+  if (fine_h < 2 || fine_w < 2 || (fine_h % 2) != 0 || (fine_w % 2) != 0 || fine_tile_rows < 2 || low_tile_rows < 1) return PXT_E_ARG;
+  const bool windowed = pts->full_w > 0;
+  if (windowed && (pts->full_h < 1 || pts->x0 < 0 || pts->y0 < 0 || pts->x0 + fine_w > pts->full_w || pts->y0 + fine_h > pts->full_h))
+    return PXT_E_ARG;
+  RefPoints rp;
+  rp.p3d = pts->p3d; rp.n = pts->n_points;
+  for (int i = 0; i < 12; ++i) rp.T[i] = pts->T[i];
+  for (int i = 0; i < 10; ++i) rp.cam[i] = pts->cam[i];
+  rp.ndist = pts->ndist; rp.pad = (float)pts->pad;
+  rp.x0 = windowed ? pts->x0 : 0; rp.y0 = windowed ? pts->y0 : 0;
+  rp.fw = windowed ? pts->full_w : fine_w; rp.fh = windowed ? pts->full_h : fine_h;
+  rp.W = fine_w; rp.H = fine_h;
+  const int low_h = fine_h / 2, low_w = fine_w / 2;
+  const RefTileGeo fine{fine_tile_rows, (fine_w + 15) / 16, (fine_h + fine_tile_rows - 1) / fine_tile_rows};
+  const RefTileGeo low{low_tile_rows, (low_w + 15) / 16, (low_h + low_tile_rows - 1) / low_tile_rows};
+  std::memset(fine_flags_host, 0, (size_t)fine.tiles_x * fine.tiles_y);
+  std::memset(low_flags_host, 0, (size_t)low.tiles_x * low.tiles_y);
+  for (int n = 0; n < rp.n; ++n) reference_tiles_mark(rp, n, fine, fine_flags_host);
+  for (int i = 0; i < fine.tiles_x * fine.tiles_y; ++i)
+    reference_tiles_spread(i, fine, fine_flags_host, low, low_h, low_w, low_flags_host);
   return PXT_OK;
 }
 
@@ -1268,15 +1420,27 @@
   return PXT_OK;
 }
 
+extern "C" int pxt_unet_forward_sampled(pxt_unet* ctx, const void* image, int32_t image_is_u8, const uint8_t* mask,
+                                        int32_t H, int32_t W, float* const out_maps[3], const int32_t out_cstride[3],
+                                        int32_t normalize, void* workspace, void* stream,
+                                        const pxt_unet_sample_points* points_host) {
+  if (!out_maps) return PXT_E_ARG;
+  const void* images[1] = {image};
+  const uint8_t* masks[1] = {mask};
+  if (!ctx || ctx->f32 || !points_host)
+    return pxt_unet_forward_batch(ctx, 1, images, &image_is_u8, masks, H, W, out_maps, out_cstride, &normalize, workspace,
+                                  stream);
+  if (ctx->join_pending) { PXT_HIP_CHECK(hipStreamWaitEvent((hipStream_t)stream, ctx->ev_join, 0)); ctx->join_pending = false; }
+  return forward_pass(ctx, 1, images, &image_is_u8, masks, H, W, out_maps, out_cstride, &normalize, workspace, stream,
+                      ctx->sides[0], PlanScope{1, false, 0}, points_host);
+}
+
 extern "C" int pxt_unet_forward(pxt_unet* ctx, const void* image, int32_t image_is_u8,
                                 const uint8_t* mask, int32_t H, int32_t W, float* const out_maps[3],
                                 const int32_t out_cstride[3], int32_t normalize, void* workspace,
                                 void* stream) {
-  if (!out_maps) return PXT_E_ARG;
-  const void* images[1] = {image};
-  const uint8_t* masks[1] = {mask};
-  return pxt_unet_forward_batch(ctx, 1, images, &image_is_u8, masks, H, W, out_maps, out_cstride, &normalize,
-                                workspace, stream);
+  return pxt_unet_forward_sampled(ctx, image, image_is_u8, mask, H, W, out_maps, out_cstride, normalize, workspace, stream,
+                                  nullptr);
 }
 
 extern "C" int pxt_unet_activation_stats(pxt_unet* ctx, int32_t H, int32_t W, const void* workspace, float* stats,
diff --git a/pixtrack_amd/feature_extractor.py b/pixtrack_amd/feature_extractor.py
--- a/pixtrack_amd/feature_extractor.py
+++ b/pixtrack_amd/feature_extractor.py
@@ -93,8 +93,13 @@
             img = dst
         return img, mask, scale_resize
 
+    def _arm(self, sample_points) -> None:
+        arm = getattr(self.model, "arm_sample_points", None)
+        if sample_points is not None and arm is not None:
+            arm(sample_points)
+
     def extract_packed(self, image, scale_image: int = 1, mask: Optional[torch.Tensor] = None,
-                       normalize: bool = False):
+                       normalize: bool = False, sample_points=None):
         for k, r in enumerate(self._preloaded):
             if r[0] is image and r[1] == scale_image and r[2] is mask and r[3] == normalize:
                 del self._preloaded[k]
@@ -109,6 +114,8 @@
         a_img, a_mask, a_sr = self._prepare(image, scale_image, mask)
         self.last_input_wh = (int(a_img.shape[1]), int(a_img.shape[0]))
         scales = [(a_sr[0] / s, a_sr[1] / s) for s in self.model.scales]
+        if sample_points is not None and (a_sr != (1.0, 1.0) or tuple(a_img.shape[:2]) != tuple(image.shape[:2])):
+            sample_points = None
         if self._staged is not None:
             st_image, st_scale, st_mask, st_norm = self._staged
             self._staged = None
@@ -117,6 +124,7 @@
                 if self.defer_join:
                     self.model.set_defer_join(True)
                 try:
+                    self._arm(sample_points)
                     both = self.model.forward_packed_batch([(a_img, a_mask, normalize), (b_img, b_mask, st_norm)])
                 finally:
                     if self.defer_join:
@@ -125,6 +133,7 @@
                 self._ready = (st_image, st_scale, st_mask, st_norm, both[1],
                                [(b_sr[0] / s, b_sr[1] / s) for s in self.model.scales], b_img, b_mask)
                 return both[0], scales
+        self._arm(sample_points)
         return self.model.forward_packed(a_img, a_mask, normalize=normalize), scales
 
     @torch.no_grad()
diff --git a/pixtrack_amd/ops.py b/pixtrack_amd/ops.py
--- a/pixtrack_amd/ops.py
+++ b/pixtrack_amd/ops.py
@@ -39,7 +39,8 @@
         "(Tensor fmap, int channels, float[] camera, int ndist, Tensor p3d, Tensor fref, Tensor? valid, Tensor poses, "
         "Tensor ranges, int pad, int loss, float loss_alpha, float loss_scale, Tensor(a!) out) -> ()"),
     "unet_forward_batch": (
-        "(int ctx, Tensor[] images, Tensor?[] masks, bool[] normalize, Tensor(a!)[] outs, Tensor(b!) workspace) -> ()"),
+        "(int ctx, Tensor[] images, Tensor?[] masks, bool[] normalize, Tensor(a!)[] outs, Tensor(b!) workspace, "
+        "Tensor? sample_p3d=None, float[]? sample_pose_camera=None, int[]? sample_ints=None) -> ()"),
     "ngp_render": (
         "(int ctx, float[] view, int width, int height, int spp, int mode, Tensor(a!) out, Tensor(b!)? stats) -> ()"),
     "ngp_render_both": (
@@ -388,9 +389,24 @@
                                            out.data_ptr(), _stream(fmap)), "pxt_score_pose_hypotheses")
 
 
-def _unet_forward_batch(ctx, images, masks, normalize, outs, workspace):
+def _unet_forward_batch(ctx, images, masks, normalize, outs, workspace, sample_p3d=None, sample_pose_camera=None,
+                        sample_ints=None):
     L = _lib.lib()
     n = len(images)
+    points = None
+    if sample_p3d is not None:
+        if n > 2 or sample_pose_camera is None or sample_ints is None or len(sample_pose_camera) != 22 or len(sample_ints) != 6:
+            raise _lib.PxtError("unet_forward_batch: sample points go with one image or a pair, 22 floats (pose, camera) "
+                                "and 6 ints (ndist, pad, x0, y0, full_w, full_h)")
+        _f32c(sample_p3d, "sample_p3d")
+        _lib.require_gpu(sample_p3d, "sample_p3d")
+        if sample_p3d.dim() != 2 or sample_p3d.shape[1] != 3 or sample_p3d.device != images[0].device:
+            raise _lib.PxtError("unet_forward_batch: sample_p3d is [N, 3] on the images' device")
+        points = _lib.UnetSamplePoints()
+        points.p3d, points.n_points = sample_p3d.data_ptr(), int(sample_p3d.shape[0])
+        points.T[:] = [float(x) for x in sample_pose_camera[:12]]
+        points.cam[:] = [float(x) for x in sample_pose_camera[12:]]
+        points.ndist, points.pad, points.x0, points.y0, points.full_w, points.full_h = (int(x) for x in sample_ints)
     if n == 0 or len(masks) != n or len(normalize) != n or len(outs) != 3 * n:
         raise _lib.PxtError("unet_forward_batch: per image one mask slot, one normalize flag and three output maps")
     sizes = [(int(im.shape[0]), int(im.shape[1])) for im in images]
@@ -418,7 +434,14 @@
     norm = (C.c_int32 * n)(*[int(bool(x)) for x in normalize])
     ptrs = (C.c_void_p * (3 * n))(*[o.data_ptr() for o in outs])
     cs = (C.c_int32 * 3)(*[int(o.shape[2]) for o in outs[:3]])
-    if pair:
+    if points is not None and n == 1:
+        _lib.check(L.pxt_unet_forward_sampled(ctx, imgs[0], is_u8[0], mks[0], H, W, ptrs, cs, norm[0], workspace.data_ptr(),
+                                              _stream(images[0]), C.byref(points)), "pxt_unet_forward_sampled")
+    elif points is not None:
+        pp = (C.POINTER(_lib.UnetSamplePoints) * 2)(C.pointer(points), None)
+        _lib.check(L.pxt_unet_forward_pair_sampled(ctx, imgs, is_u8, mks, Hs, Ws, ptrs, cs, norm, workspace.data_ptr(),
+                                                   _stream(images[0]), pp), "pxt_unet_forward_pair_sampled")
+    elif pair:
         _lib.check(L.pxt_unet_forward_pair(ctx, imgs, is_u8, mks, Hs, Ws, ptrs, cs, norm, workspace.data_ptr(),
                                            _stream(images[0])), "pxt_unet_forward_pair")
     else:
diff --git a/pixtrack_amd/refiner.py b/pixtrack_amd/refiner.py
--- a/pixtrack_amd/refiner.py
+++ b/pixtrack_amd/refiner.py
@@ -207,14 +207,44 @@
         for dbid in (dbids if dbids is not None else list(self.model3d.dbs)):
             self._points_of([int(dbid)])
 
-    def dense_feature_extraction(self, image, name: str, image_scale: int = 1, mask=None, normalize=False):
-        maps, scales = self.feature_extractor.extract_packed(image, image_scale, mask, normalize)
-        if self.tracker is not None and getattr(self.tracker, "debug", 0) >= 2:
+    def dense_feature_extraction(self, image, name: str, image_scale: int = 1, mask=None, normalize=False,
+                                 sample_points=None):
+        log_dense = self.tracker is not None and getattr(self.tracker, "debug", 0) >= 2
+        if sample_points is not None and not log_dense:
+            maps, scales = self.feature_extractor.extract_packed(image, image_scale, mask, normalize, sample_points)
+        else:
+            maps, scales = self.feature_extractor.extract_packed(image, image_scale, mask, normalize)
+        if log_dense:
             feats = [m[..., :c].permute(2, 0, 1) for m, c in zip(maps, OUTPUT_DIMS)]
             weight = [m[..., c : c + 1].permute(2, 0, 1) for m, c in zip(maps, OUTPUT_DIMS)]
             self.log_dense(name=name, image=image, image_scale=image_scale, features=feats, scales=scales,
                            weight=weight)
         return maps, scales
+
+    def _level_windows(self, window, n_levels: int):
+        if window is None:
+            return None
+        x0, y0, fw, fh = window
+        windows = []
+        for level, stride in zip(range(n_levels), self.feature_extractor.model.scales):
+            lh, lw = self.feature_extractor.model.level_shapes(fh, fw)[level]
+            windows += [x0 // stride, y0 // stride, lw, lh]
+        return windows
+
+    def reference_sample_points(self, image_id: int, pose: Pose, p3d: torch.Tensor, image, image_scale: int, window):
+        if not hasattr(image, "shape") or int(p3d.shape[0]) < 1:
+            return None
+        H, W = int(image.shape[0]), int(image.shape[1])
+        h_new, w_new, scale_resize = self.feature_extractor.target_size(H, W, image_scale)
+        if (h_new, w_new) != (H, W):
+            return None
+        camera = self._reference_camera_of(self.model3d.dbs[image_id].camera_id)
+        s0 = self.feature_extractor.model.scales[0]
+        cam_l = camera.scale((scale_resize[0] / s0, scale_resize[1] / s0))
+        pad = self.optimizer[0].interpolator.pad
+        windows = self._level_windows(window, 1) or [0, 0, 0, 0]
+        return {"p3d": p3d, "pose_camera": pose.as12().detach().cpu().reshape(-1).tolist() + cam_l.as10().tolist(),
+                "ints": [int(cam_l._data.shape[-1] - 6), int(pad)] + [int(x) for x in windows]}
 
     def interp_sparse_observations(self, feature_maps: List[torch.Tensor], feature_scales, image_id: int,
                                    p3dids: List[int], pose: Optional[Pose] = None,
@@ -234,13 +264,7 @@
         valid = torch.empty(n, dtype=torch.uint8, device=self.device)
         pad = self.optimizer[0].interpolator.pad
         T12 = T_w2cam.as12().detach().cpu().reshape(-1).tolist()
-        windows = None
-        if window is not None:
-            x0, y0, fw, fh = window
-            windows = []
-            for fm, stride in zip(feature_maps, self.feature_extractor.model.scales):
-                lh, lw = self.feature_extractor.model.level_shapes(fh, fw)[len(windows) // 4]
-                windows += [x0 // stride, y0 // stride, lw, lh]
+        windows = self._level_windows(window, len(feature_maps))
         ops.sample_sparse(p3d, T12, list(feature_maps), list(OUTPUT_DIMS[:len(feature_maps)]), cams, ndist, int(pad),
                           True, outs, valid, windows)
         return SparseReferenceFeatures(outs, valid, list(p3dids), p3d, OUTPUT_DIMS)
@@ -267,7 +291,9 @@
         features = {}
         for image_scale in multiscales:
             image, window = (reference_image, None) if render_points else self.reference_window(dbids, pose, reference_image)
-            maps, scales = self.dense_feature_extraction(image, ref_img.name, image_scale)
+            sample_points = None if render_points else self.reference_sample_points(dbids[0], pose, p3d, image, image_scale,
+                                                                                    window)
+            maps, scales = self.dense_feature_extraction(image, ref_img.name, image_scale, sample_points=sample_points)
             self.last_reference_wh = self.feature_extractor.last_input_wh
             features[str(image_scale)] = self.interp_sparse_observations(maps, scales, dbids[0], p3dids, pose, p3d, window)
             if render_points:
diff --git a/pixtrack_amd/unet.py b/pixtrack_amd/unet.py
--- a/pixtrack_amd/unet.py
+++ b/pixtrack_amd/unet.py
@@ -296,10 +296,13 @@
         return [dec[3], dec[1], (hs[4], ws[4])]
 
     def forward_packed(self, image: torch.Tensor, mask: Optional[torch.Tensor] = None,
-                       normalize: bool = False) -> List[torch.Tensor]:
+                       normalize: bool = False, sample_points=None) -> List[torch.Tensor]:
+        if sample_points is not None:
+            self.arm_sample_points(sample_points)
         return self.forward_packed_batch([(image, mask, normalize)])[0]
 
-    def forward_packed_batch(self, items) -> List[List[torch.Tensor]]:
+    def forward_packed_batch(self, items, sample_points=None) -> List[List[torch.Tensor]]:
+        armed, self._armed_points = getattr(self, "_armed_points", None), None
         n = len(items)
         sizes = [(int(it[0].shape[0]), int(it[0].shape[1])) for it in items]
         H, W = sizes[0]
@@ -316,8 +319,10 @@
             self._ws = torch.empty(need, dtype=torch.uint8, device=self.device)
         outs = [[torch.empty(h, w, cstride_for(c), device=self.device, dtype=torch.float32)
                  for (h, w), c in zip(self.level_shapes(*hw), OUTPUT_DIMS)] for hw in sizes]
+        sp = (sample_points if sample_points is not None else armed) if n <= 2 else None
         ops.unet_forward_batch(int(self._ctx.value), [it[0] for it in items], [it[1] for it in items],
-                               [bool(it[2]) for it in items], [o for per in outs for o in per], self._ws)
+                               [bool(it[2]) for it in items], [o for per in outs for o in per], self._ws,
+                               *((sp["p3d"], sp["pose_camera"], sp["ints"]) if sp else ()))
         return outs
 
     def set_batch_plan(self, per_image_plan: bool) -> None:
@@ -325,6 +330,12 @@
 
     def set_tile_skip(self, on: bool) -> None:
         _lib.check(_lib.lib().pxt_unet_set_tile_skip(self._ctx, int(bool(on))), "pxt_unet_set_tile_skip")
+
+    def arm_sample_points(self, sample_points) -> None:
+        self._armed_points = sample_points
+
+    def set_reference_tiles(self, on: bool) -> None:
+        _lib.check(_lib.lib().pxt_unet_set_reference_tiles(self._ctx, int(bool(on))), "pxt_unet_set_reference_tiles")
 
     def set_defer_join(self, on: bool) -> None:
         _lib.check(_lib.lib().pxt_unet_set_defer_join(self._ctx, int(bool(on))), "pxt_unet_set_defer_join")
```

After: 754.3 (median of 6 runs). 1.7% higher.
